# Mirko-Nava/BayesianNeuralNetworks

Measured on AMD Instinct MI355X. Metric: MC-samples/sec (node), 784-1200-1200-10 BayesianLinear MLP, batch 512, higher is better.
Workload: dtype bf16

## Files before the change

### bayesianneuralnetworks_amd/_lib.py

```python
import ctypes
import os

import torch

_HERE = os.path.dirname(os.path.abspath(__file__))
LIB_PATH = os.environ.get("BNN_HIP_LIB") or os.path.join(_HERE, "libbnn_hip.so")

F32, BF16, BF16X3 = 0, 1, 2
DRAW_FLIPOUT = 16
COMPUTE_F32, COMPUTE_BF16 = 0, 1
FLAG_RELU = 1
FLAG_X_BF16 = 2
E_ALIGN, E_UNSUPPORTED, E_DEVICE = -4, -6, -7
FLAG_Y_BF16 = 4
UNC_LOGITS, UNC_PROBS = 0, 1


class BnnHipError(RuntimeError):
    pass


ABI_VERSION = 2


class Rng(ctypes.Structure):
    _fields_ = [("seed", ctypes.c_uint64),
                ("stream", ctypes.c_uint32),
                ("sample0", ctypes.c_uint32),
                ("epoch_host", ctypes.c_uint32),
                ("epoch_dev_delta", ctypes.c_int32),
                ("epoch_dev", ctypes.c_void_p),
                ("generator", ctypes.c_uint32),
                ("reserved", ctypes.c_uint32)]


class KlTensor(ctypes.Structure):
    _fields_ = [("mu", ctypes.c_void_p),
                ("rho", ctypes.c_void_p),
                ("n", ctypes.c_int64),
                ("prior_mu", ctypes.c_float),
                ("prior_sigma", ctypes.c_float)]


class AdamTensor(ctypes.Structure):
    _fields_ = [("p", ctypes.c_void_p), ("g", ctypes.c_void_p), ("m", ctypes.c_void_p), ("v", ctypes.c_void_p),
                ("n", ctypes.c_int64)]


class KlFuse(ctypes.Structure):
    _fields_ = [("upstream", ctypes.c_void_p), ("mu_w", ctypes.c_void_p), ("mu_b", ctypes.c_void_p),
                ("scale_w", ctypes.c_float), ("prior_mu_w", ctypes.c_float), ("prior_sigma_w", ctypes.c_float),
                ("scale_b", ctypes.c_float), ("prior_mu_b", ctypes.c_float), ("prior_sigma_b", ctypes.c_float)]


class DrawTensor(ctypes.Structure):
    _fields_ = [("mu", ctypes.c_void_p), ("rho", ctypes.c_void_p), ("rows", ctypes.c_int64), ("cols", ctypes.c_int64),
                ("out", ctypes.c_void_p), ("ld", ctypes.c_int64), ("out_sample_stride", ctypes.c_int64),
                ("out_dtype", ctypes.c_int), ("kind", ctypes.c_int), ("taps", ctypes.c_int), ("rng", Rng)]


class Conv2dShape(ctypes.Structure):
    _fields_ = [(n, ctypes.c_int32) for n in
                ("B", "C", "H", "W", "O", "KH", "KW", "stride_h", "stride_w", "pad_h", "pad_w",
                 "dil_h", "dil_w", "groups")]


_p = ctypes.c_void_p
_i64 = ctypes.c_int64
_int = ctypes.c_int
_f = ctypes.c_float
_rngp = ctypes.POINTER(Rng)

SIGNATURES = {
    "bnn_abi_version": (_int, []),
    "bnn_arch": (ctypes.c_char_p, []),
    "bnn_last_error": (ctypes.c_char_p, []),
    "bnn_launch_count": (ctypes.c_uint64, []),
    "bnn_set_workspace": (_int, [_int, _p, _i64]),
    "bnn_check_device": (_int, [_int, _p]),
    "bnn_sample_affine_eps": (_int, [_p, _p, _p, _p, _i64, _int, _p]),
    "bnn_sample_affine_philox": (_int, [_p, _p, _p, _i64, _int, _i64, _int, _rngp, _p]),
    "bnn_eps_philox": (_int, [_p, _i64, _int, _i64, _rngp, _p]),
    "bnn_sigma": (_int, [_p, _p, _i64, _p]),
    "bnn_sample_affine_bwd": (_int, [_p, _i64, _p, _p, _i64, _rngp, _i64, _int, _p, _p, _int, _p]),
    "bnn_rng_advance": (_int, [_p, ctypes.c_uint32, _p]),
    "bnn_prune_score": (_int, [_p, _p, _p, _i64, _p]),
    "bnn_kl_workspace_bytes": (_i64, [_int]),
    "bnn_kl_forward": (_int, [ctypes.POINTER(KlTensor), _int, _f, _p, _p, _p]),
    "bnn_kl_forward_partial": (_int, [ctypes.POINTER(KlTensor), _int, _p, _p]),
    "bnn_kl_backward": (_int, [ctypes.POINTER(KlTensor), _int, _f, _p, ctypes.POINTER(_p),
                               ctypes.POINTER(_p), _int, _p]),
    "bnn_linear_forward_sampled": (_int, [_p, _i64, _i64, _p, _p, _p, _p, _p, _i64, _i64, _i64, _i64,
                                          _i64, _int, _rngp, _rngp, _int, _int, _p]),
    "bnn_linear_forward_sampled_kl": (_int, [_p, _i64, _i64, _p, _p, _p, _p, _p, _i64, _i64, _i64, _i64,
                                             _i64, _int, _rngp, _rngp, _int, _int, ctypes.POINTER(KlTensor), _int, _p, _p]),
    "bnn_draw_multi": (_int, [ctypes.POINTER(DrawTensor), _int, _int, ctypes.POINTER(KlTensor), _int, _p, _p]),
    "bnn_dense_forward": (_int, [_p, _i64, _i64, _p, _i64, _i64, _p, _i64, _p, _i64, _i64, _i64, _i64, _i64, _int, _int, _p]),
    "bnn_dense_forward_dropout": (_int, [_p, _i64, _i64, _p, _i64, _i64, _p, _i64, _p, _i64, _i64, _i64, _i64, _i64, _int, _int,
                                         _f, _rngp, _p]),
    "bnn_mc_dropout": (_int, [_p, _i64, _p, _i64, _i64, _i64, _int, _f, _int, _rngp, _p]),
    "bnn_flipout_signs": (_int, [_p, _i64, _i64, _i64, _int, _rngp, _p]),
    "bnn_flipout_weight_backward": (_int, [_p, _i64, _p, _p, _p, _i64, _i64, _int, _rngp, _p]),
    "bnn_mc_dropout_backward": (_int, [_p, _i64, _p, _i64, _i64, _i64, _int, _f, _int, _rngp, _p]),
    "bnn_dense_head_parts": (_int, [_i64, _i64, _int]),
    "bnn_dense_forward_head": (_int, [_p, _i64, _i64, _p, _i64, _i64, _p, _i64, _p, _i64, _i64, _p, _i64, _i64,
                                      _p, _i64, _i64, _i64, _int, _int, _p]),
    "bnn_dense_forward_x3_head": (_int, [_p, _i64, _i64, _i64, _p, _i64, _i64, _i64, _p, _i64, _p, _i64, _i64, _i64,
                                         _p, _i64, _i64, _p, _i64, _i64, _i64, _int, _int, _p]),
    "bnn_dense_forward_x3": (_int, [_p, _i64, _i64, _i64, _p, _i64, _i64, _i64, _p, _i64, _p, _i64, _i64, _i64,
                                    _i64, _i64, _i64, _int, _int, _p]),
    "bnn_split_bf16x3": (_int, [_p, _i64, _i64, _i64, _p, _i64, _i64, _p]),
    "bnn_transpose_bf16": (_int, [_p, _i64, _i64, _p, _i64, _i64, _i64, _i64, _int, _p]),
    "bnn_conv2d_dense_forward_x3": (_int, [_p, _i64, _p, _i64, _i64, _i64, _p, _i64, _p, _i64, ctypes.POINTER(Conv2dShape), _int, _int, _p]),
    "bnn_conv2d_dense_forward": (_int, [_p, _i64, _p, _i64, _i64, _p, _i64, _p, _i64, ctypes.POINTER(Conv2dShape), _int, _int, _p]),
    "bnn_conv2d_flipout_forward": (_int, [_p, _p, _i64, _p, _p, _p, ctypes.POINTER(Conv2dShape), _int, _p]),
    "bnn_conv2d_flipout_forward_mc": (_int, [_p, _i64, _p, _i64, _p, _i64, ctypes.POINTER(Conv2dShape), _int, _rngp, _int, _p]),
    "bnn_conv2d_flipout_forward_x3": (_int, [_p, _p, _i64, _i64, _p, _p, _p, ctypes.POINTER(Conv2dShape), _int, _p]),
    "bnn_linear_forward": (_int, [_p, _i64, _i64, _p, _i64, _p, _i64, _p, _i64, _i64, _i64, _i64, _i64,
                                  _int, _int, _int, _p]),
    "bnn_linear_backward_input_sampled": (_int, [_p, _i64, _i64, _p, _p, _p, _i64, _i64, _i64, _i64, _i64, _int,
                                                 _rngp, _int, _int, _p]),
    "bnn_linear_backward_input": (_int, [_p, _i64, _i64, _p, _i64, _p, _i64, _i64, _i64, _i64, _i64, _int, _int, _p]),
    "bnn_linear_backward_weight_sampled": (_int, [_p, _i64, _i64, _p, _i64, _i64, _p, _p, _p, _p, _p, _p, _i64, _i64,
                                                  _i64, _int, _rngp, _rngp, ctypes.POINTER(KlFuse), _int, _int, _int, _p]),
    "bnn_linear_backward_narrow_sampled": (_int, [_p, _i64, _i64, _p, _i64, _i64, _p, _p, _p, _i64, _i64, _p, _p, _p, _p, _p,
                                                  _i64, _i64, _i64, _int, _rngp, _rngp, ctypes.POINTER(KlFuse), _int, _int, _p]),
    "bnn_linear_backward_weight": (_int, [_p, _i64, _i64, _p, _i64, _i64, _p, _i64, _i64, _i64, _i64, _int, _int,
                                          _int, _int, _p]),
    "bnn_colsum": (_int, [_p, _i64, _i64, _p, _i64, _i64, _int, _int, _p]),
    "bnn_relu_backward": (_int, [_p, _p, _p, _i64, _int, _p]),
    "bnn_adam_step": (_int, [ctypes.POINTER(AdamTensor), _int, _f, _f, _f, _f, _f, _p, _p]),
    "bnn_adam_step_advance": (_int, [ctypes.POINTER(AdamTensor), _int, _f, _f, _f, _f, _f, _p, _p, ctypes.c_uint32, _p]),
    "bnn_xent_workspace_bytes": (_i64, [_i64]),
    "bnn_softmax_xent": (_int, [_p, _p, _i64, _int, _p, _p, _p, _p]),
    "bnn_conv2d_im2col": (_int, [_p, _i64, ctypes.POINTER(Conv2dShape), _int, _p, _int, _p]),
    "bnn_conv2d_col2im": (_int, [_p, ctypes.POINTER(Conv2dShape), _int, _int, _p, _p]),
    "bnn_nchw_to_rows": (_int, [_p, _i64, _int, _int, _p, _int, _p]),
    "bnn_conv2d_workspace_bytes": (_i64, [ctypes.POINTER(Conv2dShape), _int, _int]),
    "bnn_conv2d_forward_sampled": (_int, [_p, _i64, _p, _p, _p, _p, _p, _i64,
                                          ctypes.POINTER(Conv2dShape), _int, _rngp, _rngp, _int, _int, _p, _i64, _p]),
    "bnn_conv2d_forward": (_int, [_p, _i64, _p, _i64, _p, _i64, _p, _i64, ctypes.POINTER(Conv2dShape),
                                  _int, _int, _int, _p, _i64, _p]),
    "bnn_diag_sampler": (_int, [_p, _int, _int, _int, _p]),
    "bnn_diag_astream": (_int, [_p, _int, _int, _int, _int, _int, _int, _int, _p, _p]),
    "bnn_mc_sum": (_int, [_p, _i64, _int, _i64, _f, _p, _int, _p, ctypes.c_uint32, _p]),
    "bnn_mc_sum_kl": (_int, [_p, _i64, _int, _i64, _f, _p, _int, _p, ctypes.c_uint32, ctypes.POINTER(KlTensor), _int, _f,
                             _p, _p, _p]),
    "bnn_mc_uncertainty": (_int, [_p, _i64, _int, _int, _i64, _int, _int, _p, _p, _p, _p, _p, ctypes.c_uint32,
                                  ctypes.POINTER(KlTensor), _int, _f, _p, _p, _p]),
}

_lib = None


def load():
    global _lib
    if _lib is not None:
        return _lib
    if not os.path.exists(LIB_PATH):
        raise BnnHipError(
            "libbnn_hip.so is not built (%s). Run `python -c 'import __graft_entry__ as g; g.build()'` "
            "or `make -C bayesianneuralnetworks_amd/csrc`. There is no fallback path." % LIB_PATH)
    try:
        lib = ctypes.CDLL(LIB_PATH)
    except OSError as e:
        raise BnnHipError("cannot load %s: %s" % (LIB_PATH, e))
    for name, (res, args) in SIGNATURES.items():
        fn = getattr(lib, name)
        fn.restype = res
        fn.argtypes = args
    if lib.bnn_abi_version() != ABI_VERSION:
        raise BnnHipError("libbnn_hip.so has ABI version %d, this package binds version %d (bnn_rng_t carries the generator id "
                          "since version 2): rebuild with `make -C bayesianneuralnetworks_amd/csrc`" % (lib.bnn_abi_version(), ABI_VERSION))
    _lib = _DeviceGuarded(lib)
    return _lib


class _StreamPtr(ctypes.c_void_p):
    device_index = None


class _DeviceGuarded:

    def __init__(self, lib):
        self._lib = lib

    def __getattr__(self, name):
        fn = getattr(self._lib, name)

        def call(*args):
            st = args[-1] if args else None
            if isinstance(st, _StreamPtr) and st.device_index is not None and st.device_index != torch.cuda.current_device():
                with torch.cuda.device(st.device_index):
                    return fn(*args)
            return fn(*args)

        call.__name__ = name
        setattr(self, name, call)
        return call


_workspaces = {}


def ensure_workspace(device):
    idx = device.index if device.index is not None else torch.cuda.current_device()
    if idx not in _workspaces:
        ws = torch.zeros(4 << 20, dtype=torch.uint8, device=torch.device("cuda", idx))
        torch.cuda.synchronize(idx)
        check(load().bnn_set_workspace(idx, ctypes.c_void_p(ws.data_ptr()), ws.numel()), "bnn_set_workspace")
        _workspaces[idx] = ws
    return _workspaces[idx]


def check(rc, what):
    if rc != 0:
        msg = load().bnn_last_error().decode("utf-8", "replace")
        raise BnnHipError("%s failed (code %d): %s" % (what, rc, msg))


def stream_ptr(device=None):
    sp = _StreamPtr(torch.cuda.current_stream(device).cuda_stream)
    if device is not None:
        d = torch.device(device)
        sp.device_index = d.index if d.index is not None else torch.cuda.current_device()
    return sp


def check_device(device=None):
    d = torch.device("cuda", torch.cuda.current_device()) if device is None else torch.device(device)
    idx = d.index if d.index is not None else torch.cuda.current_device()
    check(load().bnn_check_device(idx, stream_ptr(torch.device("cuda", idx))), "bnn_check_device")


def ptr(t):
    if t is None:
        return None
    return ctypes.c_void_p(t.data_ptr())


def require_cuda_act(t, name, contiguous=True):
    if not t.is_cuda:
        raise BnnHipError("%s must be a CUDA/HIP tensor" % name)
    if t.dtype not in (torch.float32, torch.bfloat16):
        raise BnnHipError("%s must be float32 or bfloat16, got %s" % (name, t.dtype))
    if contiguous and not t.is_contiguous():
        raise BnnHipError("%s must be contiguous" % name)


def require_cuda_f32(t, name):
    if not t.is_cuda:
        raise BnnHipError("%s must be a CUDA/HIP tensor" % name)
    if t.dtype != torch.float32:
        raise BnnHipError("%s must be float32, got %s" % (name, t.dtype))
    if not t.is_contiguous():
        raise BnnHipError("%s must be contiguous" % name)
```

### bayesianneuralnetworks_amd/csrc/bnn_dense.hip

```cpp
#include <cstdlib>
#include <type_traits>

#include "bnn_device.hpp"
#include "bnn_dma.hpp"
#include "bnn_kl_body.hpp"

namespace bnn {

typedef float f32x4 __attribute__((ext_vector_type(4)));
typedef __bf16 bf16x8 __attribute__((ext_vector_type(8)));

constexpr int kDrawMaxTensors = 8;
constexpr int kDrawSpreadBelow = 4096;

struct DrawTensorDev {
    const float *mu;
    const float *rho;
    void *out;
    int64_t out_sample_stride;
    int32_t rows, cols, ld;
    int32_t bf16;
    int32_t kind;
    int32_t perm_taps;
    int32_t first_item;
    int32_t spread;
    int32_t flat, pad_first;
    int32_t tapg;
    int32_t kl_on, kl_first;
    float kl_prior_mu, kl_prior_sigma;
    RngDev rng;
};
struct DrawLaunch {
    DrawTensorDev t[kDrawMaxTensors];
    int32_t ntensors;
    int32_t nsamples;
    int32_t total_items;
    int32_t draw_blocks;
    KlPiggy kl;
};

template <int U, bool LEAN>
__device__ __forceinline__ void draw_multi_body(const DrawLaunch &L);

template <int U>
__global__ __launch_bounds__(256) void k_draw_multi(const DrawLaunch L) { draw_multi_body<U, false>(L); }

__global__ __launch_bounds__(256) void k_draw_lean(const DrawLaunch L) { draw_multi_body<1, true>(L); }

template <int U, bool LEAN>
__device__ __forceinline__ void draw_multi_body(const DrawLaunch &L)
{
    if ((int)blockIdx.x < L.kl.nblocks) {
        if (blockIdx.y == 0) kl_piggy_block(L.kl, (int)blockIdx.x);
        return;
    }
    const int item0 = ((int)blockIdx.x - L.kl.nblocks) * 256;
    int ti = 0;
#pragma unroll
    for (int i = 1; i < kDrawMaxTensors; ++i)
        if (i < L.ntensors && item0 >= L.t[i].first_item) ti = i;
    ti = __builtin_amdgcn_readfirstlane(ti);
    const float *const t_mu = L.t[ti].mu;
    const float *const t_rho = L.t[ti].rho;
    char *const t_out = reinterpret_cast<char *>(L.t[ti].out);
    const int64_t t_stride = L.t[ti].out_sample_stride;
    const int t_rows = L.t[ti].rows, t_cols = L.t[ti].cols, t_ld = L.t[ti].ld;
    const bool t_bf16 = L.t[ti].bf16 != 0;
    const bool t_x3 = !LEAN && L.t[ti].bf16 == 2;
    const int t_taps = L.t[ti].perm_taps;
    const int t_kind = L.t[ti].kind;
    const RngDev rng = L.t[ti].rng;
    const int S = L.nsamples;
    int local = item0 + (int)threadIdx.x - L.t[ti].first_item;
    if (L.t[ti].flat) {
        const int esz2 = 2;
        const int64_t sbytes2 = t_stride * esz2, pbytes2 = sbytes2 * S;
        const int padg = (t_ld - t_cols) >> 3;
        if (item0 >= L.t[ti].pad_first) {
            const int pi = item0 + (int)threadIdx.x - L.t[ti].pad_first;
            const int prow = pi / (padg > 0 ? padg : 1);
            if (padg == 0 || prow >= t_rows) return;
            char *d0 = t_out + ((int64_t)prow * t_ld + t_cols + ((pi - prow * padg) << 3)) * esz2;
            for (int s = (int)blockIdx.y; s < S; s += (int)gridDim.y)
                for (int pl = 0; pl < (t_x3 ? 3 : 1); ++pl) *reinterpret_cast<uint4 *>(d0 + s * sbytes2 + pl * pbytes2) = make_uint4(0u, 0u, 0u, 0u);
            return;
        }
        const int64_t e0 = (int64_t)local * 8;
        const bool live = e0 < (int64_t)t_rows * t_cols;
        const uint32_t edev = rng_epoch_dev(rng);
        float4 m0 = make_float4(0.f, 0.f, 0.f, 0.f), m1 = m0, r0 = m0, r1 = m0;
        if (live) {
            m0 = *reinterpret_cast<const float4 *>(t_mu + e0); m1 = *reinterpret_cast<const float4 *>(t_mu + e0 + 4);
            r0 = *reinterpret_cast<const float4 *>(t_rho + e0); r1 = *reinterpret_cast<const float4 *>(t_rho + e0 + 4);
        }
        if (L.t[ti].kl_on && blockIdx.y == 0) {
            const float inv_ps = __uint_as_float(uniform_vgpr(__float_as_uint(1.0f / L.t[ti].kl_prior_sigma)));
            const float pmu = __uint_as_float(uniform_vgpr(__float_as_uint(L.t[ti].kl_prior_mu)));
            float acc = 0.f;
            if (live) {
                acc += kl_elem(m0.x, r0.x, pmu, inv_ps); acc += kl_elem(m0.y, r0.y, pmu, inv_ps);
                acc += kl_elem(m0.z, r0.z, pmu, inv_ps); acc += kl_elem(m0.w, r0.w, pmu, inv_ps);
                acc += kl_elem(m1.x, r1.x, pmu, inv_ps); acc += kl_elem(m1.y, r1.y, pmu, inv_ps);
                acc += kl_elem(m1.z, r1.z, pmu, inv_ps); acc += kl_elem(m1.w, r1.w, pmu, inv_ps);
            }
            kl_block_reduce(acc, L.t[ti].kl_first + ((item0 - L.t[ti].first_item) >> 8), L.kl.partials);
        }
        if (!live) return;
        const int gpc = t_cols >> 3;
        const int row = local / gpc, c0 = (local - row * gpc) << 3;
        const float m[8] = {m0.x, m0.y, m0.z, m0.w, m1.x, m1.y, m1.z, m1.w};
        const float sg[8] = {sigma_draw(r0.x), sigma_draw(r0.y), sigma_draw(r0.z), sigma_draw(r0.w),
                             sigma_draw(r1.x), sigma_draw(r1.y), sigma_draw(r1.z), sigma_draw(r1.w)};
        const PhiloxKeys keys = philox_keys(rng.key0, rng.key1);
        const uint32_t blk = (uint32_t)(e0 >> 2);
        const bool gen16 = LEAN || rng.gen == BNN_GEN_PHILOX7_U16;
        char *dst = t_out + ((int64_t)row * t_ld + c0) * esz2 + (int64_t)blockIdx.y * sbytes2;
        const int64_t step = sbytes2 * (int64_t)gridDim.y;
#pragma unroll U
        for (int s = (int)blockIdx.y; s < S; s += (int)gridDim.y, dst += step) {
            const uint32_t sample = rng.sample0 + (uint32_t)s;
            float4 za, zb;
            if (gen16) {
                eps8_u16(rng, keys, edev, blk >> 1, sample, za, zb);
            } else {
                za = eps4(rng, keys, edev, blk, sample);
                zb = eps4(rng, keys, edev, blk + 1u, sample);
            }
            float w[8];
            w[0] = fmaf(sg[0], za.x, m[0]); w[1] = fmaf(sg[1], za.y, m[1]);
            w[2] = fmaf(sg[2], za.z, m[2]); w[3] = fmaf(sg[3], za.w, m[3]);
            w[4] = fmaf(sg[4], zb.x, m[4]); w[5] = fmaf(sg[5], zb.y, m[5]);
            w[6] = fmaf(sg[6], zb.z, m[6]); w[7] = fmaf(sg[7], zb.w, m[7]);
            if (t_x3) {
                uint4 h, mm, l;
                split_bf16x3(w[0], w[1], h.x, mm.x, l.x); split_bf16x3(w[2], w[3], h.y, mm.y, l.y);
                split_bf16x3(w[4], w[5], h.z, mm.z, l.z); split_bf16x3(w[6], w[7], h.w, mm.w, l.w);
                *reinterpret_cast<uint4 *>(dst) = h;
                *reinterpret_cast<uint4 *>(dst + pbytes2) = mm;
                *reinterpret_cast<uint4 *>(dst + 2 * pbytes2) = l;
            } else {
                uint4 o;
                o.x = pack_bf16x2(w[0], w[1]); o.y = pack_bf16x2(w[2], w[3]);
                o.z = pack_bf16x2(w[4], w[5]); o.w = pack_bf16x2(w[6], w[7]);
                *reinterpret_cast<uint4 *>(dst) = o;
            }
        }
        return;
    }
    if (!LEAN && L.t[ti].tapg) {
        __shared__ __attribute__((aligned(16))) uint16_t timg[3][256 * 8];
        const int taps = t_taps;
        const int ng = 2048 / (8 * taps);
        const int Cn = t_cols / taps, C8 = Cn >> 3;
        const int NG = t_rows * C8;
        const int g0 = ((item0 - L.t[ti].first_item) >> 8) * ng;
        const int i = (int)threadIdx.x;
        const int gl = i / taps, b = i - gl * taps;
// ... 1172 lines not shown
                }
            }
        };
        using I0 = std::integral_constant<int, 0>;
        using I1 = std::integral_constant<int, 1>;
        if (nk_run > 0) {
            __builtin_amdgcn_s_barrier();
            asm volatile("" ::: "memory");
            rd(I0{}, I0{});
            for (int kt = 0; kt + 1 < nk_run; ++kt) {
                rd(I1{}, I1{});
                mm(I0{});
                __builtin_amdgcn_sched_barrier(0);
                asm volatile("s_waitcnt lgkmcnt(0)" ::: "memory");
                __builtin_amdgcn_s_barrier();
                asm volatile("" ::: "memory");
                rd(I0{}, I0{});
                mm(I1{});
                __builtin_amdgcn_sched_barrier(0);
            }
            rd(I1{}, I1{});
            mm(I0{});
            mm(I1{});
        }
    }

    __syncthreads();
    float *T = reinterpret_cast<float *>(lds);
    if constexpr (KEYED) {
        const float *rs = reinterpret_cast<const float *>(lds + LDSB) - NSX * p.IMG * p.O;
#pragma unroll
        for (int n = 0; n < NSX; ++n) {
            if (n >= nvalid) break;
            if (n > 0) __syncthreads();
            if (wave < NWV) {
#pragma unroll
                for (int b = 0; b < TO; ++b) {
                    const int o = b * 16 + fi;
#pragma unroll
                    for (int a = 0; a < TM; ++a) {
                        const int row0 = wave * WM + a * 16 + fq * 4;
                        int il = row0 / P, pix = row0 - il * P;
#pragma unroll
                        for (int r = 0; r < 4; ++r) {
                            if (row0 + r < imgs * P && o < p.O)
                                T[(il * p.O + o) * P + pix] = fmaf(rs[(n * p.IMG + il) * p.O + o], acc[a][TO + n * TO + b][r], acc[a][b][r]);
                            if (++pix == P) { pix = 0; ++il; }
                        }
                    }
                }
            }
            __syncthreads();
            float *Yt = p.Y + (int64_t)(s + n) * p.y_sample_stride + (int64_t)b0 * p.O * P;
            const int nn = (p.flags & 4) ? 0 : imgs * p.O * P;
            if ((nn & 3) == 0 && (reinterpret_cast<uintptr_t>(Yt) & 15u) == 0) {
                for (int i = tid; i < (nn >> 2); i += 512) reinterpret_cast<uint4 *>(Yt)[i] = reinterpret_cast<const uint4 *>(T)[i];
            } else {
                for (int i = tid; i < nn; i += 512) Yt[i] = T[i];
            }
        }
        return;
    }
    if (wave < NWV) {
        const float *bias = p.bias ? p.bias + (int64_t)s * p.bias_sample_stride : nullptr;
#pragma unroll
        for (int b = 0; b < NOUT / 16; ++b) {
            const int o = b * 16 + fi;
            const float bv = (bias && o < p.O) ? bias[o] : 0.f;
#pragma unroll
            for (int a = 0; a < TM; ++a) {
                const int row0 = wave * WM + a * 16 + fq * 4;
                int il = row0 / P, pix = row0 - il * P;
#pragma unroll
                for (int r = 0; r < 4; ++r) {
                    if (row0 + r < imgs * P && o < p.O) {
                        float v = acc[a][b][r] + bv;
                        if constexpr (FLIP) v = fmaf(p.sgn_out[(int64_t)(b0 + il) * p.O + o], acc[a][b + TN / 2][r], v);
                        T[(il * p.O + o) * P + pix] = v;
                    }
                    if (++pix == P) { pix = 0; ++il; }
                }
            }
        }
    }
    __syncthreads();
    {
        float *Yt = p.Y + (int64_t)s * p.y_sample_stride + (int64_t)b0 * p.O * P;
        const int n = (p.flags & 4) ? 0 : imgs * p.O * P;
        if ((n & 3) == 0 && (reinterpret_cast<uintptr_t>(Yt) & 15u) == 0) {
            for (int i = tid; i < (n >> 2); i += 512) reinterpret_cast<uint4 *>(Yt)[i] = reinterpret_cast<const uint4 *>(T)[i];
        } else {
            for (int i = tid; i < n; i += 512) Yt[i] = T[i];
        }
    }
}

static inline bool al16(const void *q) { return (reinterpret_cast<uintptr_t>(q) & 15u) == 0; }

}

using namespace bnn;

namespace bnn {
__global__ __launch_bounds__(256) void k_split_bf16x3(const float *__restrict__ x, int gpr, int64_t ldx, uint16_t *__restrict__ out,
                                                     int64_t ld_out, int64_t plane_stride, int items)
{
    const int i = (int)(blockIdx.x * 256 + threadIdx.x);
    if (i >= items) return;
    const int row = i / gpr, c0 = (i - row * gpr) * 8;
    const float4 a = *reinterpret_cast<const float4 *>(x + (int64_t)row * ldx + c0);
    const float4 b = *reinterpret_cast<const float4 *>(x + (int64_t)row * ldx + c0 + 4);
    uint4 h, m, l;
    split_bf16x3(a.x, a.y, h.x, m.x, l.x);
    split_bf16x3(a.z, a.w, h.y, m.y, l.y);
    split_bf16x3(b.x, b.y, h.z, m.z, l.z);
    split_bf16x3(b.z, b.w, h.w, m.w, l.w);
    uint16_t *o = out + (int64_t)row * ld_out + c0;
    *reinterpret_cast<uint4 *>(o) = h;
    *reinterpret_cast<uint4 *>(o + plane_stride) = m;
    *reinterpret_cast<uint4 *>(o + 2 * plane_stride) = l;
}

__global__ __launch_bounds__(256) void k_transpose_bf16(const uint16_t *__restrict__ in, int64_t in_batch_stride, int64_t ld_in,
                                                       uint16_t *__restrict__ out, int64_t out_batch_stride, int64_t ld_out,
                                                       int rows, int cols)
{
    constexpr int PITCH = 72;
    __shared__ __attribute__((aligned(16))) uint16_t T[64 * PITCH];
    const int r0 = (int)blockIdx.x * 64, c0 = (int)blockIdx.y * 64;
    const uint16_t *src = in + (int64_t)blockIdx.z * in_batch_stride;
    uint16_t *dst = out + (int64_t)blockIdx.z * out_batch_stride;
#pragma unroll
    for (int j = 0; j < 2; ++j) {
        const int q = (int)threadIdx.x + 256 * j;
        const int r = q >> 3, cc = (q & 7) * 8;
        uint4 v = make_uint4(0u, 0u, 0u, 0u);
        if (r0 + r < rows && c0 + cc < cols) v = *reinterpret_cast<const uint4 *>(src + (int64_t)(r0 + r) * ld_in + c0 + cc);
        const uint32_t e[4] = {v.x, v.y, v.z, v.w};
#pragma unroll
        for (int i = 0; i < 4; ++i) {
            T[(cc + 2 * i) * PITCH + r] = (uint16_t)(e[i] & 0xFFFFu);
            T[(cc + 2 * i + 1) * PITCH + r] = (uint16_t)(e[i] >> 16);
        }
    }
    __syncthreads();
#pragma unroll
    for (int j = 0; j < 2; ++j) {
        const int q = (int)threadIdx.x + 256 * j;
        const int c = q >> 3, rc = (q & 7) * 8;
        if (c0 + c < cols && r0 + rc < ld_out)
            *reinterpret_cast<uint4 *>(dst + (int64_t)(c0 + c) * ld_out + r0 + rc) = *reinterpret_cast<const uint4 *>(&T[c * PITCH + rc]);
    }
}
}

struct HeadArgs {
    const void *wh;
    int64_t wh_plane_stride;
    int64_t wh_sample_stride, ldwh;
    const float *bh;
    int64_t bh_sample_stride;
    float *partials;
    int64_t nh;
};

struct DropArgs {
    float p;
    const bnn_rng_t *rng;
    bool fan;
};

static int dense_pick_tile(int64_t M, int64_t N, int nsamples)
{
    static const int force_tile = [] { const char *e = getenv("BNN_DENSE_TILE"); return e ? atoi(e) : -1; }();
    int tile = (N % 80 == 0 || N < 128) ? 1 : 2;
    if (N <= 80) tile = 0;
    if (force_tile >= 0 && force_tile <= 4) tile = force_tile;
    if (tile == 1 && force_tile < 0) {
        const int64_t cols = (N + 159) / 160;
        if (((M + 127) / 128) * cols * nsamples < 128 && M > 64) tile = 3;
        if (tile == 3 && ((M + 63) / 64) * cols * nsamples < 128 && M > 32) tile = 4;
    }
    return tile;
}

static int dense_launch(const char *who, const void *x, int64_t x_plane_stride, int64_t x_sample_stride, int64_t ldx,
                        const void *w, int64_t w_plane_stride, int64_t w_sample_stride, int64_t ldw,
                        const float *b, int64_t b_sample_stride,
                        void *y, int64_t y_plane_stride, int64_t y_sample_stride, int64_t ldy,
                        int64_t M, int64_t N, int64_t K, int nsamples, int flags, bool x3, void *stream, const HeadArgs *head = nullptr,
                        const DropArgs *drop = nullptr)
{
    if (M == 0 && N >= 1 && K >= 1 && nsamples >= 1) return BNN_OK;
    if (head) { y = head->partials; ldy = N; }
    if (!x || !w || !y) { set_error("%s: NULL pointer", who); return BNN_E_NULL; }
    if (M < 0 || N < 1 || K < 1 || nsamples < 1 || ldx < K || ldy < N) { set_error("%s: bad extent", who); return BNN_E_SHAPE; }
    if (M > 0x7FFFFFFF || N > 0x7FFFFFFF || K > 0x7FFFFFFF) { set_error("%s: extent too large", who); return BNN_E_RANGE; }
    if (flags & ~(BNN_FLAG_RELU | BNN_FLAG_Y_BF16)) { set_error("%s: unknown flags", who); return BNN_E_UNSUPPORTED; }
    const int64_t kp = (K + 63) / 64 * 64;
    if (K % 8 != 0 || ldx % 8 != 0 || x_sample_stride % 8 != 0 || ldw % 8 != 0 || w_sample_stride % 8 != 0 || ldw < kp || !al16(x) || !al16(w)) {
        set_error("%s: needs K %% 8 == 0, 16-B aligned bf16 rows, and weight rows zero-padded to ldw >= roundup(K, 64)", who);
        return BNN_E_UNSUPPORTED;
    }
    if (M * ldx * 2 >= ((int64_t)1 << 32) || N * ldw * 2 >= ((int64_t)1 << 32)) { set_error("%s: one sample's operand exceeds 4 GiB", who); return BNN_E_RANGE; }
    const bool ybf = (flags & BNN_FLAG_Y_BF16) != 0;
    if (reinterpret_cast<uintptr_t>(y) & (ybf ? 1u : 3u)) { set_error("%s: misaligned output", who); return BNN_E_ALIGN; }
    DenseParams p{};
    p.A = reinterpret_cast<const uint16_t *>(x); p.a_sample_stride = x_sample_stride; p.lda = ldx;
    p.W = reinterpret_cast<const uint16_t *>(w); p.w_sample_stride = w_sample_stride; p.ldw = ldw;
    p.bias = b; p.bias_sample_stride = b_sample_stride;
    p.Y = y; p.y_sample_stride = y_sample_stride; p.ldy = ldy;
    p.M = (int32_t)M; p.N = (int32_t)N; p.K = (int32_t)K; p.S = nsamples; p.flags = flags;
    if (x3) {
        if (x_plane_stride % 8 != 0 || w_plane_stride % 8 != 0 || (ybf && y_plane_stride % 8 != 0) || x_plane_stride < M * ldx || w_plane_stride < N * ldw) {
            set_error("%s: bad plane stride", who);
            return BNN_E_SHAPE;
        }
        if (N <= 16 && (K > 4 * kHeadMaxSteps * 32 || ybf)) { set_error("%s: a narrow layer (N <= 16) on three-plane operands needs K <= %d and fp32 outputs", who, 4 * kHeadMaxSteps * 32); return BNN_E_UNSUPPORTED; }
        p.x3 = 1;
        p.a_plane_stride = x_plane_stride; p.w_plane_stride = w_plane_stride; p.y_plane_stride = y_plane_stride;
    }
    if (head) {
        if (N <= 16 || (flags & BNN_FLAG_Y_BF16) == 0) { set_error("%s: the fused head follows a hidden layer wider than 16", who); return BNN_E_UNSUPPORTED; }
        if (x3 && (head->wh_plane_stride % 8 != 0 || head->wh_plane_stride < head->nh * head->ldwh)) { set_error("%s: bad plane stride of the head's weights", who); return BNN_E_SHAPE; }
        if (x3) {
            const int t_ = dense_pick_tile(M, N, nsamples);
            if (t_ == 0 || t_ == 2) { set_error("%s: the three-plane fused head runs on the 160-column tiles (N %% 80 == 0 or N < 128, N > 80)", who); return BNN_E_UNSUPPORTED; }
        }
        if (!head->wh || head->nh < 1 || head->nh > 16) { set_error("%s: head of 1 .. 16 outputs", who); return BNN_E_SHAPE; }
        if (N % 8 != 0 || head->ldwh % 8 != 0 || head->ldwh < N || head->wh_sample_stride % 8 != 0 || !al16(head->wh) ||
            (reinterpret_cast<uintptr_t>(head->partials) & 3u)) {
            set_error("%s: the head's weights need N %% 8 == 0 and 16-B aligned rows zero-padded to ldwh >= N", who);
            return BNN_E_UNSUPPORTED;
        }
        p.Wh = reinterpret_cast<const uint16_t *>(head->wh); p.wh_sample_stride = head->wh_sample_stride; p.ldwh = head->ldwh;
        p.bias_h = head->bh; p.bias_h_sample_stride = head->bh_sample_stride;
        p.P = head->partials; p.Nh = (int32_t)head->nh;
        p.wh_plane_stride = head->wh_plane_stride;
    }
    hipStream_t st = (hipStream_t)stream;
    const int full_samples = nsamples;
    if (drop) {
        if (x3 || head) { set_error("%s: the dropout epilogue takes plain bf16 operands", who); return BNN_E_UNSUPPORTED; }
        p.drop_rng = make_rng(drop->rng);
        p.drop_p = drop->p;
        p.drop_scale = drop->p < 1.f ? 1.f / (1.f - drop->p) : 0.f;
        p.drop_fan = drop->fan ? nsamples : 1;
        if (drop->fan) nsamples = p.S = 1;
    }
    if (N <= 16 && K <= 4 * kHeadMaxSteps * 32) {
        p.ntm = (int32_t)((M + 15) / 16);
        p.ntn = 1;
        hipLaunchKernelGGL(k_head_bf16, dim3((unsigned)((int64_t)p.ntm * nsamples)), dim3(256), 0, st, p);
        int rc = check_launch(who);
        if (rc == BNN_OK && drop)
            rc = mc_dropout_launch(who, y, drop->fan ? 0 : y_sample_stride, ldy, y, y_sample_stride, ldy, M, N, full_samples, drop->fan,
                                   drop->p, ybf ? BNN_BF16 : BNN_F32, drop->rng, st);
        return rc;
    }
    const bool fused_drop = drop && N % 4 == 0;
    static const bool no_xcd = [] { const char *e = getenv("BNN_DENSE_XCD"); return e && e[0] == '0'; }();
    if (no_xcd) p.flags |= kDenseNoXcdMap;
    static const bool lprio = [] { const char *e = getenv("BNN_DENSE_LOADER_PRIO"); return e && e[0] == '1'; }();
    if (lprio) p.flags |= kDenseLoaderPrio;
    int tile = dense_pick_tile(M, N, nsamples);
    if (fused_drop && tile == 2) tile = 1;
    const int bm = tile == 1 ? 128 : tile == 3 ? 64 : tile == 4 ? 32 : 256;
    const int bn = tile == 0 ? 80 : tile == 2 ? 128 : 160;
    p.ntm = (int32_t)((M + bm - 1) / bm);
    p.ntn = (int32_t)((N + bn - 1) / bn);
    const int64_t grid = (int64_t)p.ntm * p.ntn * nsamples;
    if (grid > 0x7FFFFFFF) { set_error("%s: grid too large", who); return BNN_E_RANGE; }
    static const int diag = [] { const char *e = getenv("BNN_DENSE_DIAG"); return e ? atoi(e) : 0; }();
    if (diag >= 6 && diag <= 9 && !head && !drop) {
        static const uint64_t stamps = [] { const char *e = getenv("BNN_DENSE_STAMPS"); return e ? strtoull(e, nullptr, 0) : 0ull; }();
        p.P = reinterpret_cast<float *>(stamps);
    }
    const bool relu = (flags & BNN_FLAG_RELU) != 0;
    const dim3 g((unsigned)grid), blk(512);
#define BNN_DENSE_LAUNCH(TM_, TN_, NWM_, NWN_, ST_, RELU_, DROP_) \
    do { \
        if (fused_drop && ybf) hipLaunchKernelGGL((k_dense_bf16<TM_, TN_, NWM_, NWN_, ST_, 1, RELU_, 0, DROP_>), g, blk, 0, st, p); \
        else if (fused_drop) hipLaunchKernelGGL((k_dense_bf16<TM_, TN_, NWM_, NWN_, ST_, 0, RELU_, 0, DROP_>), g, blk, 0, st, p); \
        else if (head) hipLaunchKernelGGL((k_dense_bf16<TM_, TN_, NWM_, NWN_, ST_, 3, RELU_>), g, blk, 0, st, p); \
        else if (x3 && ybf) hipLaunchKernelGGL((k_dense_bf16<TM_, TN_, NWM_, NWN_, ST_, 2, RELU_>), g, blk, 0, st, p); \
        else if (!ybf) hipLaunchKernelGGL((k_dense_bf16<TM_, TN_, NWM_, NWN_, ST_, 0, RELU_>), g, blk, 0, st, p); \
        else if (diag == 1) hipLaunchKernelGGL((k_dense_bf16<TM_, TN_, NWM_, NWN_, ST_, 1, RELU_, 1>), g, blk, 0, st, p); \
        else if (diag == 2) hipLaunchKernelGGL((k_dense_bf16<TM_, TN_, NWM_, NWN_, ST_, 1, RELU_, 2>), g, blk, 0, st, p); \
        else if (diag == 3) hipLaunchKernelGGL((k_dense_bf16<TM_, TN_, NWM_, NWN_, ST_, 1, RELU_, 3>), g, blk, 0, st, p); \
        else if (diag == 4) hipLaunchKernelGGL((k_dense_bf16<TM_, TN_, NWM_, NWN_, ST_, 1, RELU_, 4>), g, blk, 0, st, p); \
        else if (diag == 5) hipLaunchKernelGGL((k_dense_bf16<TM_, TN_, NWM_, NWN_, ST_, 1, RELU_, 5>), g, blk, 0, st, p); \
        else if (diag == 6) hipLaunchKernelGGL((k_dense_bf16<TM_, TN_, NWM_, NWN_, ST_, 1, RELU_, 6>), g, blk, 0, st, p); \
        else if (diag == 7) hipLaunchKernelGGL((k_dense_bf16<TM_, TN_, NWM_, NWN_, ST_, 1, RELU_, 7>), g, blk, 0, st, p); \
        else if (diag == 8) hipLaunchKernelGGL((k_dense_bf16<TM_, TN_, NWM_, NWN_, ST_, 1, RELU_, 8>), g, blk, 0, st, p); \
        else if (diag == 9) hipLaunchKernelGGL((k_dense_bf16<TM_, TN_, NWM_, NWN_, ST_, 1, RELU_, 9>), g, blk, 0, st, p); \
        else hipLaunchKernelGGL((k_dense_bf16<TM_, TN_, NWM_, NWN_, ST_, 1, RELU_>), g, blk, 0, st, p); \
    } while (0)
#define BNN_DENSE_PICK(TM_, TN_, NWM_, NWN_, ST_, DROP_) \
    do { \
        if (relu) BNN_DENSE_LAUNCH(TM_, TN_, NWM_, NWN_, ST_, true, DROP_); else BNN_DENSE_LAUNCH(TM_, TN_, NWM_, NWN_, ST_, false, DROP_); \
    } while (0)
    if (tile == 0) BNN_DENSE_PICK(4, 5, 4, 1, 3, true);
    else if (tile == 1) BNN_DENSE_PICK(4, 5, 2, 2, 4, true);
    else if (tile == 3) BNN_DENSE_PICK(2, 5, 2, 2, 4, true);
    else if (tile == 4) BNN_DENSE_PICK(1, 5, 2, 2, 4, true);
    else BNN_DENSE_PICK(4, 8, 4, 1, 3, false);
#undef BNN_DENSE_PICK
#undef BNN_DENSE_LAUNCH
    int rc = check_launch(who);
    if (rc == BNN_OK && drop && !fused_drop)
        rc = mc_dropout_launch(who, y, drop->fan ? 0 : y_sample_stride, ldy, y, y_sample_stride, ldy, M, N, full_samples, drop->fan,
                               drop->p, ybf ? BNN_BF16 : BNN_F32, drop->rng, st);
    return rc;
}


extern "C" {

int bnn_draw_multi(const bnn_draw_tensor_t *tensors, int ntensors, int nsamples,
                   const bnn_kl_tensor_t *kl_tensors, int kl_ntensors, void *kl_workspace, void *stream)
{
    const char *who = "bnn_draw_multi";
    if (!tensors) { set_error("%s: NULL tensors", who); return BNN_E_NULL; }
    if (ntensors < 1 || ntensors > kDrawMaxTensors) { set_error("%s: 1 .. %d tensors per call", who, kDrawMaxTensors); return BNN_E_RANGE; }
    if (nsamples < 1) { set_error("%s: nsamples < 1", who); return BNN_E_SHAPE; }
    DrawLaunch L{};
    L.ntensors = ntensors;
    L.nsamples = nsamples;
    int64_t items = 0;
    for (int i = 0; i < ntensors; ++i) {
        const bnn_draw_tensor_t &t = tensors[i];
        if (!t.mu || !t.rho || !t.out) { set_error("%s: tensor %d: NULL pointer", who, i); return BNN_E_NULL; }
        if (t.rows < 1 || t.cols < 1 || t.ld < t.cols || t.rows > 0x7FFFFFFF || t.ld > 0x7FFFFFFF) { set_error("%s: tensor %d: bad extent", who, i); return BNN_E_SHAPE; }
        if (t.out_dtype != BNN_F32 && t.out_dtype != BNN_BF16 && t.out_dtype != BNN_BF16X3) { set_error("%s: tensor %d: unknown dtype", who, i); return BNN_E_DTYPE; }
        if (t.rows > 1 && t.cols % 4 != 0) { set_error("%s: tensor %d: cols %% 4 != 0 (use bnn_sample_affine_philox)", who, i); return BNN_E_UNSUPPORTED; }
        if (t.ld % 8 != 0 && t.rows > 1) { set_error("%s: tensor %d: ld %% 8 != 0", who, i); return BNN_E_UNSUPPORTED; }
        if (t.out_dtype != BNN_F32 && (!al16(t.out) || t.out_sample_stride % 8 != 0 || t.ld % 8 != 0)) { set_error("%s: tensor %d: bf16 output needs 16-B aligned rows", who, i); return BNN_E_ALIGN; }
        if ((reinterpret_cast<uintptr_t>(t.mu) | reinterpret_cast<uintptr_t>(t.rho) | reinterpret_cast<uintptr_t>(t.out)) & 3u) { set_error("%s: tensor %d: misaligned pointer", who, i); return BNN_E_ALIGN; }
        const int rc = (t.kind == 0 || t.kind == BNN_DRAW_FLIPOUT) ? check_rng(&t.rng, nsamples) : BNN_OK;
        if (rc) { set_error("%s: tensor %d: bad rng", who, i); return rc; }
        DrawTensorDev &d = L.t[i];
        d.mu = t.mu; d.rho = t.rho; d.out = t.out; d.out_sample_stride = t.out_sample_stride;
        d.rows = (int32_t)t.rows; d.cols = (int32_t)t.cols; d.ld = (int32_t)t.ld; d.bf16 = t.out_dtype == BNN_BF16 ? 1 : t.out_dtype == BNN_BF16X3 ? 2 : 0;
        d.perm_taps = t.taps > 1 ? t.taps : 1;
        d.kind = t.kind;
        if ((t.kind < 0 || t.kind > 3) && t.kind != BNN_DRAW_FLIPOUT) { set_error("%s: tensor %d: kind must be 0 (draw), 1 (mean), 2 (stddev), 3 (as it is, once) or BNN_DRAW_FLIPOUT", who, i); return BNN_E_RANGE; }
        if (t.kind == BNN_DRAW_FLIPOUT && (t.taps > 1 || t.out_dtype == BNN_BF16X3 || t.rows + t.cols > 0xFFFFFFFFll)) { set_error("%s: tensor %d: a Flipout draw is a linear weight (no taps, fp32 or bf16 output, rows + cols < 2^32)", who, i); return BNN_E_SHAPE; }
        if (t.taps > 1 && (t.cols % t.taps != 0 || t.out_dtype == BNN_F32)) { set_error("%s: tensor %d: taps must divide cols (bf16 or three-plane output)", who, i); return BNN_E_SHAPE; }
        d.first_item = (int32_t)items;
        d.rng = make_rng(&t.rng);
        const int64_t nit = t.rows * ((t.ld + 7) / 8);
        d.spread = (nit < kDrawSpreadBelow && nsamples > 1 && nit * nsamples <= 0x7FFFFFFF) ? 1 : 0;
        d.flat = (!d.spread && t.out_dtype != BNN_F32 && t.kind == 0 && t.taps <= 1 && t.cols % 8 == 0 && t.ld % 8 == 0 && al16(t.mu) && al16(t.rho)) ? 1 : 0;
        d.tapg = (t.taps > 1 && t.taps <= 256 && t.out_dtype != BNN_F32 && t.rows >= 1 && (t.cols / t.taps) % 8 == 0 && t.ld % 8 == 0 &&
                  al16(t.mu) && (t.kind == 1 || t.kind == 3 || al16(t.rho))) ? 1 : 0;
        static const bool no_tapg = [] { const char *e = getenv("BNN_DRAW_TAPG"); return e && e[0] == '0'; }();
        if (no_tapg) d.tapg = 0;
        if (d.tapg) {
            d.spread = 0;
            const int64_t ng = 2048 / (8 * t.taps), NG = t.rows * (t.cols / t.taps / 8);
            items += (NG + ng - 1) / ng * 256;
        } else if (d.flat) {
            items += (t.rows * (t.cols / 8) + 255) / 256 * 256;
            d.pad_first = (int32_t)items;
            items += (t.rows * ((t.ld - t.cols) / 8) + 255) / 256 * 256;
        } else
        items += ((d.spread ? nit * nsamples : nit) + 255) / 256 * 256;
        if (items > 0x7FFFFF00) { set_error("%s: too many elements for one call", who); return BNN_E_RANGE; }
    }
    L.total_items = (int32_t)items;
    L.draw_blocks = (int32_t)((items + 255) / 256);
    int64_t grid = L.draw_blocks;
    if (kl_tensors && kl_ntensors > 0) {
        if (!kl_plan_piggy(kl_tensors, kl_ntensors, kl_workspace, L.kl)) {
            set_error("%s: the KL first pass cannot ride along (more than %d tensors, bad prior or no workspace): launch bnn_kl_forward_partial", who, kKlPiggyMax);
            return BNN_E_UNSUPPORTED;
        }
        static const bool kl_items = [] { const char *e = getenv("BNN_DRAW_KL_ITEMS"); return !(e && e[0] == '0'); }();
        int32_t launched = 0;
        for (int j = 0; j < kl_ntensors; ++j) {
            const int32_t nb = L.kl.pg_first[j + 1] - L.kl.pg_first[j];
            bool in_items = false;
            for (int i = 0; i < ntensors && kl_items && !in_items; ++i) {
                DrawTensorDev &d = L.t[i];
                if (d.flat && !d.kl_on && d.mu == kl_tensors[j].mu && d.rho == kl_tensors[j].rho &&
                    kl_tensors[j].n == (int64_t)d.rows * d.cols) {
                    d.kl_on = 1; d.kl_first = L.kl.t[j].first_block;
                    d.kl_prior_mu = kl_tensors[j].prior_mu; d.kl_prior_sigma = kl_tensors[j].prior_sigma;
                    in_items = true;
                }
            }
            L.kl.pg_first[j] = launched;
            if (!in_items) launched += nb;
        }
        L.kl.pg_first[kl_ntensors] = launched;
        L.kl.nblocks = launched;
        grid += L.kl.nblocks;
    }
    int split = 1;
    while (split < nsamples && (int64_t)L.draw_blocks * split < 1024) split *= 2;
    if (split > nsamples) split = nsamples;
    static const int force_split = [] { const char *e = getenv("BNN_DRAW_SPLIT"); return e ? atoi(e) : 0; }();
    if (force_split >= 1 && force_split <= nsamples) split = force_split;
    static const int unroll = [] { const char *e = getenv("BNN_DRAW_UNROLL"); return e ? atoi(e) : 1; }();
    bool lean = true;
    for (int i = 0; i < ntensors; ++i) {
        const DrawTensorDev &d = L.t[i];
        if (d.tapg || d.perm_taps > 1 || d.bf16 == 2 || d.kind == BNN_DRAW_FLIPOUT || (d.kind == 0 && d.rng.gen != BNN_GEN_PHILOX7_U16)) lean = false;
    }
    static const bool no_lean = [] { const char *e = getenv("BNN_DRAW_LEAN"); return e && e[0] == '0'; }();
    if (lean && !no_lean && unroll <= 1) hipLaunchKernelGGL(k_draw_lean, dim3((unsigned)grid, (unsigned)split), dim3(256), 0, (hipStream_t)stream, L);
    else if (unroll == 2) hipLaunchKernelGGL(k_draw_multi<2>, dim3((unsigned)grid, (unsigned)split), dim3(256), 0, (hipStream_t)stream, L);
    else if (unroll == 4) hipLaunchKernelGGL(k_draw_multi<4>, dim3((unsigned)grid, (unsigned)split), dim3(256), 0, (hipStream_t)stream, L);
    else if (unroll == 8) hipLaunchKernelGGL(k_draw_multi<8>, dim3((unsigned)grid, (unsigned)split), dim3(256), 0, (hipStream_t)stream, L);
    else
    hipLaunchKernelGGL(k_draw_multi<1>, dim3((unsigned)grid, (unsigned)split), dim3(256), 0, (hipStream_t)stream, L);
    return check_launch(who);
}

int bnn_dense_forward(const void *x, int64_t x_sample_stride, int64_t ldx,
                      const void *w, int64_t w_sample_stride, int64_t ldw,
                      const float *b, int64_t b_sample_stride,
                      void *y, int64_t y_sample_stride, int64_t ldy,
                      int64_t M, int64_t N, int64_t K, int nsamples, int flags, void *stream)
{
    return dense_launch("bnn_dense_forward", x, 0, x_sample_stride, ldx, w, 0, w_sample_stride, ldw, b, b_sample_stride,
                        y, 0, y_sample_stride, ldy, M, N, K, nsamples, flags, false, stream);
}

int bnn_dense_forward_dropout(const void *x, int64_t x_sample_stride, int64_t ldx,
                              const void *w, int64_t w_sample_stride, int64_t ldw,
                              const float *b, int64_t b_sample_stride,
                              void *y, int64_t y_sample_stride, int64_t ldy,
                              int64_t M, int64_t N, int64_t K, int nsamples, int flags, float p, const bnn_rng_t *rng, void *stream)
{
    const char *who = "bnn_dense_forward_dropout";
    if (!x || !w || !y) { set_error("%s: NULL pointer", who); return BNN_E_NULL; }
    int rc = check_dropout_args(who, M, N, nsamples, p, rng);
    if (rc) return rc;
    if (x_sample_stride < 0 || w_sample_stride < 0 || b_sample_stride < 0 || y_sample_stride < 0 ||
        (nsamples > 1 && y_sample_stride < (M - 1) * ldy + N)) { set_error("%s: bad sample stride", who); return BNN_E_SHAPE; }
    const DropArgs d{p, rng, x_sample_stride == 0 && w_sample_stride == 0 && (b == nullptr || b_sample_stride == 0)};
    return dense_launch(who, x, 0, x_sample_stride, ldx, w, 0, w_sample_stride, ldw, b, b_sample_stride,
                        y, 0, y_sample_stride, ldy, M, N, K, nsamples, flags, false, stream, nullptr, &d);
}

int bnn_dense_head_parts(int64_t M, int64_t N, int nsamples)
{
    if (M < 1 || N < 17 || nsamples < 1) return 0;
    const int tile = dense_pick_tile(M, N, nsamples);
    const int bn = tile == 0 ? 80 : tile == 2 ? 128 : 160;
    const int nwn = (tile == 0 || tile == 2) ? 1 : 2;
    return (int)((N + bn - 1) / bn) * nwn;
}

int bnn_dense_forward_head(const void *x, int64_t x_sample_stride, int64_t ldx,
                           const void *w, int64_t w_sample_stride, int64_t ldw,
                           const float *b, int64_t b_sample_stride,
                           const void *w_head, int64_t wh_sample_stride, int64_t ldwh,
                           const float *b_head, int64_t bh_sample_stride, int64_t n_head,
                           float *partials, int64_t M, int64_t N, int64_t K, int nsamples, int flags, void *stream)
{
    HeadArgs h{w_head, 0, wh_sample_stride, ldwh, b_head, bh_sample_stride, partials, n_head};
    return dense_launch("bnn_dense_forward_head", x, 0, x_sample_stride, ldx, w, 0, w_sample_stride, ldw, b, b_sample_stride,
                        nullptr, 0, 0, N, M, N, K, nsamples, flags | BNN_FLAG_Y_BF16, false, stream, &h);
}

int bnn_dense_forward_x3_head(const void *x, int64_t x_plane_stride, int64_t x_sample_stride, int64_t ldx,
                              const void *w, int64_t w_plane_stride, int64_t w_sample_stride, int64_t ldw,
                              const float *b, int64_t b_sample_stride,
                              const void *w_head, int64_t wh_plane_stride, int64_t wh_sample_stride, int64_t ldwh,
                              const float *b_head, int64_t bh_sample_stride, int64_t n_head,
                              float *partials, int64_t M, int64_t N, int64_t K, int nsamples, int flags, void *stream)
{
    if (wh_plane_stride <= 0) { set_error("bnn_dense_forward_x3_head: plane stride of the head's weights"); return BNN_E_SHAPE; }
    HeadArgs h{w_head, wh_plane_stride, wh_sample_stride, ldwh, b_head, bh_sample_stride, partials, n_head};
    return dense_launch("bnn_dense_forward_x3_head", x, x_plane_stride, x_sample_stride, ldx, w, w_plane_stride, w_sample_stride, ldw,
                        b, b_sample_stride, nullptr, 0, 0, N, M, N, K, nsamples, flags | BNN_FLAG_Y_BF16, true, stream, &h);
}

int bnn_dense_forward_x3(const void *x, int64_t x_plane_stride, int64_t x_sample_stride, int64_t ldx,
                         const void *w, int64_t w_plane_stride, int64_t w_sample_stride, int64_t ldw,
                         const float *b, int64_t b_sample_stride,
                         void *y, int64_t y_plane_stride, int64_t y_sample_stride, int64_t ldy,
                         int64_t M, int64_t N, int64_t K, int nsamples, int flags, void *stream)
{
    return dense_launch("bnn_dense_forward_x3", x, x_plane_stride, x_sample_stride, ldx, w, w_plane_stride, w_sample_stride, ldw,
                        b, b_sample_stride, y, y_plane_stride, y_sample_stride, ldy, M, N, K, nsamples, flags, true, stream);
}

int bnn_split_bf16x3(const float *x, int64_t rows, int64_t cols, int64_t ldx, void *out, int64_t ld_out, int64_t plane_stride, void *stream)
{
    const char *who = "bnn_split_bf16x3";
    if (rows == 0 && cols >= 1) return BNN_OK;
    if (!x || !out) { set_error("%s: NULL pointer", who); return BNN_E_NULL; }
    if (rows < 0 || cols < 1 || ldx < cols || ld_out < cols) { set_error("%s: bad extent", who); return BNN_E_SHAPE; }
    if (cols % 8 != 0 || ldx % 4 != 0 || ld_out % 8 != 0 || plane_stride % 8 != 0 || !al16(x) || !al16(out)) {
        set_error("%s: needs cols %% 8 == 0 and 16-B aligned rows on both sides", who);
        return BNN_E_UNSUPPORTED;
    }
    const int64_t items = rows * (cols / 8);
    if (items > 0x7FFFFFFF) { set_error("%s: too many elements", who); return BNN_E_RANGE; }
    hipLaunchKernelGGL(k_split_bf16x3, dim3((unsigned)((items + 255) / 256)), dim3(256), 0, (hipStream_t)stream,
                       x, (int)(cols / 8), ldx, reinterpret_cast<uint16_t *>(out), ld_out, plane_stride, (int)items);
    return check_launch(who);
}

int bnn_transpose_bf16(const void *in, int64_t in_batch_stride, int64_t ld_in, void *out, int64_t out_batch_stride, int64_t ld_out,
                       int64_t rows, int64_t cols, int batch, void *stream)
{
    const char *who = "bnn_transpose_bf16";
    if ((rows == 0 || batch == 0) && cols >= 1) return BNN_OK;
    if (!in || !out) { set_error("%s: NULL pointer", who); return BNN_E_NULL; }
    if (rows < 0 || cols < 1 || batch < 0 || ld_in < cols || ld_out < rows) { set_error("%s: bad extent", who); return BNN_E_SHAPE; }
    if (cols % 8 != 0 || ld_in % 8 != 0 || ld_out % 8 != 0 || in_batch_stride % 8 != 0 || out_batch_stride % 8 != 0 || !al16(in) || !al16(out)) {
        set_error("%s: needs cols %% 8 == 0 and 16-B aligned rows on both sides", who);
        return BNN_E_UNSUPPORTED;
    }
    if (rows > 0x7FFFFFFF || cols > 0x7FFFFFFF || (cols + 63) / 64 > 65535 || batch > 65535) { set_error("%s: extent too large", who); return BNN_E_RANGE; }
    hipLaunchKernelGGL(k_transpose_bf16, dim3((unsigned)((ld_out + 63) / 64), (unsigned)((cols + 63) / 64), (unsigned)batch), dim3(256), 0,
                       (hipStream_t)stream, reinterpret_cast<const uint16_t *>(in), in_batch_stride, ld_in,
                       reinterpret_cast<uint16_t *>(out), out_batch_stride, ld_out, (int)rows, (int)cols);
    return check_launch(who);
}


}

static int conv_dense_launch(const float *x, int64_t x_sample_stride, const void *w, int64_t w_sample_stride, int64_t ldw,
                             const float *b, int64_t b_sample_stride, const float *sgn_in, const float *sgn_out,
                             float *y, int64_t y_sample_stride, const bnn_conv2d_shape_t *sh, int nsamples, int flags,
                             void *stream, const char *who, int64_t w_plane_stride = 0, const bnn_rng_t *rng = nullptr)
{
    const bool keyed = rng != nullptr;
    const bool flip = sgn_in != nullptr || keyed;
    const bool x3 = w_plane_stride != 0;
    if (!x || !w || !y || !sh || (flip && !keyed && !sgn_out)) { set_error("%s: NULL pointer", who); return BNN_E_NULL; }
    if (sh->B < 1 || sh->C < 1 || sh->H < 1 || sh->W < 1 || sh->O < 1 || sh->KH < 1 || sh->KW < 1 || sh->stride_h < 1 ||
        sh->stride_w < 1 || sh->pad_h < 0 || sh->pad_w < 0 || sh->dil_h < 1 || sh->dil_w < 1 || nsamples < 1) { set_error("%s: bad shape", who); return BNN_E_SHAPE; }
    if (flags != 0) { set_error("%s: unknown flags", who); return BNN_E_UNSUPPORTED; }
    const int OH = (sh->H + 2 * sh->pad_h - sh->dil_h * (sh->KH - 1) - 1) / sh->stride_h + 1;
    const int OW = (sh->W + 2 * sh->pad_w - sh->dil_w * (sh->KW - 1) - 1) / sh->stride_w + 1;
    if (OH < 1 || OW < 1) { set_error("%s: kernel larger than the padded input", who); return BNN_E_SHAPE; }
    const int K = sh->C * sh->KH * sh->KW;
    const int bn = flip ? 2 * sh->O : sh->O;
    const bool ok = sh->groups == 1 && (sh->C == 64 || sh->C % 128 == 0) && (bn == 64 || bn == 128) &&
                    ldw >= K && ldw % 8 == 0 && w_sample_stride % 8 == 0 && al16(w) &&
                    (reinterpret_cast<uintptr_t>(x) & 3u) == 0 && (reinterpret_cast<uintptr_t>(y) & 3u) == 0;
    if (!ok) { set_error("%s: needs groups = 1, C = 64 or a multiple of 128, O = 64 or 128 (Flipout: 32 or 64), tap-major bf16 weights with 16-B aligned rows", who); return BNN_E_UNSUPPORTED; }
    const int ns = !keyed ? 0 : (x_sample_stride != 0 || nsamples == 1) ? 1 : (nsamples == 2 || bn == 128) ? 2 : 4;
    if (keyed) {
        const int rc = check_flip_args(who, sh->B, (int64_t)sh->O + sh->C, nsamples, rng);
        if (rc) return rc;
    }
    ConvParams p{};
    const int64_t img_bytes = (int64_t)sh->H * sh->W * sh->C * 2 + (flip ? (sh->C / 8) * 16 * (keyed ? ns : 1) : 0);
    const int64_t rsign = keyed ? (int64_t)ns * sh->O * 4 : 0;
    const int P = OH * OW;
    if (x3 && (w_plane_stride % 8 != 0 || w_plane_stride < (int64_t)bn * ldw)) { set_error("%s: bad plane stride", who); return BNN_E_SHAPE; }
    const int st = bn == 64 ? 4 : (x3 ? 3 : flip ? 4 : 6);
    const int64_t lds_block = (bn == 64 && !x3 && !keyed) ? kConvLds : kConvLdsBig;
    const int64_t ring = (int64_t)st * bn * 128;
    int img = 128 / P;
    while (img > 0 && (img * (img_bytes * (x3 ? 3 : 1) + rsign) + ring > lds_block || (int64_t)img * (sh->O * P * 4 + rsign) > lds_block)) --img;
    if (img > sh->B) img = sh->B;
    if (img < 1 || (int64_t)bn * ldw * 2 >= ((int64_t)1 << 32)) { set_error("%s: one image (%lld B bf16) + the weight ring do not fit the LDS block, or more than 128 output pixels per image", who, (long long)img_bytes); return BNN_E_UNSUPPORTED; }
    p.X = x; p.x_sample_stride = x_sample_stride;
    p.W = reinterpret_cast<const uint16_t *>(w); p.w_sample_stride = w_sample_stride; p.ldw = ldw;
    p.bias = b; p.bias_sample_stride = b_sample_stride;
    p.Y = y; p.y_sample_stride = y_sample_stride;
    p.sgn_in = sgn_in; p.sgn_out = sgn_out;
    p.w_plane_stride = w_plane_stride;
    p.B = sh->B; p.C = sh->C; p.H = sh->H; p.Wd = sh->W; p.O = sh->O; p.KH = sh->KH; p.KW = sh->KW;
    p.sh = sh->stride_h; p.sw = sh->stride_w; p.ph = sh->pad_h; p.pw = sh->pad_w; p.dh = sh->dil_h; p.dw = sh->dil_w;
    static const int cdiag = [] { const char *e = getenv("BNN_CONV_DIAG"); return e ? atoi(e) : 0; }();
    p.flags = cdiag;
    p.OH = OH; p.OW = OW; p.S = nsamples; p.IMG = img; p.ntiles = (sh->B + img - 1) / img;
    p.img_bytes = (int32_t)((int64_t)sh->H * sh->W * sh->C * 2);
    if (keyed) p.rng = make_rng(rng);
    const int64_t grid = (int64_t)p.ntiles * (keyed ? (nsamples + ns - 1) / ns : nsamples);
    if (grid > 0x7FFFFFFF) { set_error("%s: grid too large", who); return BNN_E_RANGE; }
    const dim3 g((unsigned)grid), blk(512);
    hipStream_t stq = (hipStream_t)stream;
    if (keyed) {
        if (bn == 64) {
            if (ns == 1) hipLaunchKernelGGL((k_conv_bf16<4, 4, kConvLdsBig, true, false, 1>), g, blk, 0, stq, p);
            else if (ns == 2) hipLaunchKernelGGL((k_conv_bf16<4, 4, kConvLdsBig, true, false, 2>), g, blk, 0, stq, p);
            else hipLaunchKernelGGL((k_conv_bf16<4, 4, kConvLdsBig, true, false, 4>), g, blk, 0, stq, p);
        } else {
            if (ns == 1) hipLaunchKernelGGL((k_conv_bf16<8, 4, kConvLdsBig, true, false, 1>), g, blk, 0, stq, p);
            else hipLaunchKernelGGL((k_conv_bf16<8, 4, kConvLdsBig, true, false, 2>), g, blk, 0, stq, p);
        }
    } else if (x3 && flip) {
        if (bn == 64) hipLaunchKernelGGL((k_conv_bf16<4, 4, kConvLdsBig, true, true>), g, blk, 0, stq, p);
        else hipLaunchKernelGGL((k_conv_bf16<8, 3, kConvLdsBig, true, true>), g, blk, 0, stq, p);
    } else if (x3) {
        if (bn == 64) hipLaunchKernelGGL((k_conv_bf16<4, 4, kConvLdsBig, false, true>), g, blk, 0, stq, p);
        else hipLaunchKernelGGL((k_conv_bf16<8, 3, kConvLdsBig, false, true>), g, blk, 0, stq, p);
    } else if (flip) {
        if (bn == 64) hipLaunchKernelGGL((k_conv_bf16<4, 4, kConvLds, true>), g, blk, 0, stq, p);
        else hipLaunchKernelGGL((k_conv_bf16<8, 4, kConvLdsBig, true>), g, blk, 0, stq, p);
    } else {
        if (bn == 64) hipLaunchKernelGGL((k_conv_bf16<4, 4, kConvLds>), g, blk, 0, stq, p);
        else hipLaunchKernelGGL((k_conv_bf16<8, 6, kConvLdsBig>), g, blk, 0, stq, p);
    }
    return check_launch(who);
}

extern "C" {

int bnn_conv2d_dense_forward(const float *x, int64_t x_sample_stride,
                             const void *w, int64_t w_sample_stride, int64_t ldw,
                             const float *b, int64_t b_sample_stride,
                             float *y, int64_t y_sample_stride,
                             const bnn_conv2d_shape_t *sh, int nsamples, int flags, void *stream)
{
    return conv_dense_launch(x, x_sample_stride, w, w_sample_stride, ldw, b, b_sample_stride, nullptr, nullptr, y, y_sample_stride,
                             sh, nsamples, flags, stream, "bnn_conv2d_dense_forward");
}

int bnn_conv2d_dense_forward_x3(const float *x, int64_t x_sample_stride,
                                const void *w, int64_t w_plane_stride, int64_t w_sample_stride, int64_t ldw,
                                const float *b, int64_t b_sample_stride,
                                float *y, int64_t y_sample_stride,
                                const bnn_conv2d_shape_t *sh, int nsamples, int flags, void *stream)
{
    if (w_plane_stride <= 0) { set_error("bnn_conv2d_dense_forward_x3: plane stride"); return BNN_E_SHAPE; }
    return conv_dense_launch(x, x_sample_stride, w, w_sample_stride, ldw, b, b_sample_stride, nullptr, nullptr, y, y_sample_stride,
                             sh, nsamples, flags, stream, "bnn_conv2d_dense_forward_x3", w_plane_stride);
}

int bnn_conv2d_flipout_forward(const float *x, const void *w, int64_t ldw, const float *sign_in, const float *sign_out,
                               float *y, const bnn_conv2d_shape_t *sh, int flags, void *stream)
{
    if (!sign_in || !sign_out) { set_error("bnn_conv2d_flipout_forward: NULL sign tensor"); return BNN_E_NULL; }
    return conv_dense_launch(x, 0, w, 0, ldw, nullptr, 0, sign_in, sign_out, y, 0, sh, 1, flags, stream, "bnn_conv2d_flipout_forward");
}

int bnn_conv2d_flipout_forward_mc(const float *x, int64_t x_sample_stride, const void *w, int64_t ldw, float *y,
                                  int64_t y_sample_stride, const bnn_conv2d_shape_t *sh, int nsamples, const bnn_rng_t *rng,
                                  int flags, void *stream)
{
    const char *who = "bnn_conv2d_flipout_forward_mc";
// ... 22 lines not shown
```

### bayesianneuralnetworks_amd/csrc/bnn_gemm.hip

```cpp
#include <cstdlib>

#include "bnn_device.hpp"
#include "bnn_gemm_params.hpp"

namespace bnn {

typedef float f32x4 __attribute__((ext_vector_type(4)));
typedef __bf16 bf16x8 __attribute__((ext_vector_type(8)));

__device__ __forceinline__ int swz(int row, int chunk)
{
    return chunk ^ ((0x78 >> (((row >> 2) & 3) * 2)) & 3);
}

template <int BM, int BN, int WM, int WN, int A_MODE, int B_MODE, int COMPUTE>
__global__ __launch_bounds__(WM * WN * 64) void k_gemm_nt(const GemmParams p)
{
    constexpr int NT = WM * WN * 64;
    constexpr int KPC = (COMPUTE == BNN_COMPUTE_F32) ? 4 : 8;
    constexpr int BK = 4 * KPC;
    constexpr int WTM = BM / WM, WTN = BN / WN;
    constexpr int TM = WTM / 16, TN = WTN / 16;
    static_assert(WTM % 16 == 0 && WTN % 16 == 0, "wave tile must be a multiple of 16x16");
    constexpr int A_CHUNKS = BM * 4, B_CHUNKS = BN * 4;
// ... 177 lines not shown
                Bs[row * 4 + swz(row, c)] = pack(bm[i]);
            }
        }
    };

    f32x4 acc[TM][TN];
#pragma unroll
    for (int a = 0; a < TM; ++a)
#pragma unroll
        for (int b = 0; b < TN; ++b) acc[a][b] = f32x4{0.f, 0.f, 0.f, 0.f};

    const int nk = (p.K + BK - 1) / BK;
    const int fi = lane & 15, fq = lane >> 4;

    load_A(0);
    load_B(0);
    sample_B(0);
    store_tiles(0);
    __syncthreads();

    for (int kt = 0; kt < nk; ++kt) {
        const int buf = kt & 1;
        const bool more = kt + 1 < nk;
        if (more) {
            load_A((kt + 1) * BK);
            load_B((kt + 1) * BK);
        }
        const uint4 *As = As0 + buf * A_CHUNKS, *Bs = Bs0 + buf * B_CHUNKS;
        uint4 af[TM], bf[TN];
#pragma unroll
        for (int a = 0; a < TM; ++a) {
            const int row = wm * WTM + a * 16 + fi;
            af[a] = As[row * 4 + swz(row, fq)];
        }
#pragma unroll
        for (int b = 0; b < TN; ++b) {
            const int row = wn * WTN + b * 16 + fi;
            bf[b] = Bs[row * 4 + swz(row, fq)];
        }
        if constexpr (COMPUTE == BNN_COMPUTE_F32) {
#pragma unroll
            for (int j = 0; j < 4; ++j)
#pragma unroll
                for (int a = 0; a < TM; ++a)
#pragma unroll
                    for (int b = 0; b < TN; ++b) {
                        const uint32_t ua = j == 0 ? af[a].x : j == 1 ? af[a].y : j == 2 ? af[a].z : af[a].w;
                        const uint32_t ub = j == 0 ? bf[b].x : j == 1 ? bf[b].y : j == 2 ? bf[b].z : bf[b].w;
                        acc[a][b] = __builtin_amdgcn_mfma_f32_16x16x4f32(__uint_as_float(ua), __uint_as_float(ub),
                                                                         acc[a][b], 0, 0, 0);
                    }
        } else {
#pragma unroll
            for (int a = 0; a < TM; ++a)
#pragma unroll
                for (int b = 0; b < TN; ++b)
                    acc[a][b] = __builtin_amdgcn_mfma_f32_16x16x32_bf16(__builtin_bit_cast(bf16x8, af[a]),
                                                                        __builtin_bit_cast(bf16x8, bf[b]),
                                                                        acc[a][b], 0, 0, 0);
        }
        if (more) {
            sample_B((kt + 1) * BK);
            store_tiles(buf ^ 1);
        }
        __syncthreads();
    }

    uint32_t edev_b = 0;
    const bool sampled_bias = (p.mu_b != nullptr);
    if (sampled_bias) edev_b = rng_epoch_dev(p.rng_b);
#pragma unroll
    for (int b = 0; b < TN; ++b) {
        const int n = n0 + wn * WTN + b * 16 + fi;
        if (n >= p.N) continue;
        const int64_t ng = nrow0 + n;
        float bias = 0.f;
        if (sampled_bias)
            bias = fmaf(sigma_draw(p.rho_b[ng]), eps1(p.rng_b, edev_b, (uint64_t)ng, p.rng_b.sample0 + (uint32_t)s), p.mu_b[ng]);
        else if (p.bias)
            bias = p.bias[(int64_t)s * p.bias_sample_stride + ng];
#pragma unroll
        for (int a = 0; a < TM; ++a) {
#pragma unroll
            for (int r = 0; r < 4; ++r) {
                const int m = m0 + wm * WTM + a * 16 + fq * 4 + r;
                if (m >= p.M) continue;
                float v = acc[a][b][r] + bias;
                if (p.flags & BNN_FLAG_RELU) v = fmaxf(v, 0.f);
                float *Yb = p.Y + (int64_t)s * p.y_sample_stride;
                if constexpr (A_MODE == A_DENSE) {
                    Yb[(int64_t)m * p.ldy + ng] = v;
                } else {
                    const int hw = p.OH * p.OW;
                    const int bimg = m / hw, pix = m % hw;
                    Yb[((int64_t)bimg * p.O + ng) * hw + pix] = v;
                }
            }
        }
    }
}

struct TileCfg { int bm, bn; };

template <int BM, int BN, int WM, int WN, int AM, int BMODE, int CP>
static void launch_cfg(GemmParams &p, hipStream_t st)
{
    p.ntm = (p.M + BM - 1) / BM;
    p.ntn = (p.N + BN - 1) / BN;
    const int panels = p.ntn * p.G;
    const int64_t grid = (int64_t)8 * ((panels + 7) / 8) * p.ntm * p.S;
    hipLaunchKernelGGL((k_gemm_nt<BM, BN, WM, WN, AM, BMODE, CP>), dim3((unsigned)grid), dim3(WM * WN * 64), 0, st, p);
}

template <int AM, int BMODE, int CP>
static void launch_select(GemmParams &p, hipStream_t st)
{
    const int64_t tiles_big = (int64_t)((p.M + 255) / 256) * ((p.N + 79) / 80) * p.S * p.G;
    if (p.N <= 16) {
        launch_cfg<64, 16, 4, 1, AM, BMODE, CP>(p, st);
    } else if (p.M >= 256 && p.N >= 80 && tiles_big >= 128) {
        launch_cfg<256, 80, 8, 1, AM, BMODE, CP>(p, st);
    } else {
        launch_cfg<64, 64, 2, 2, AM, BMODE, CP>(p, st);
    }
}

template <int AM>
static int dispatch(GemmParams &p, bool sampled, int compute, hipStream_t st, const char *who)
{
    if (compute == BNN_COMPUTE_F32) {
        if (sampled) launch_select<AM, B_SAMPLED, BNN_COMPUTE_F32>(p, st);
        else launch_select<AM, B_PLAIN, BNN_COMPUTE_F32>(p, st);
    } else if (compute == BNN_COMPUTE_BF16) {
        if (sampled) launch_select<AM, B_SAMPLED, BNN_COMPUTE_BF16>(p, st);
        else launch_select<AM, B_PLAIN, BNN_COMPUTE_BF16>(p, st);
    } else {
        set_error("%s: unknown compute mode %d", who, compute);
        return BNN_E_DTYPE;
    }
    return check_launch(who);
}

static void *g_ws[64];
static int64_t g_ws_bytes[64];
constexpr int64_t kTicketBytes = 64 * 1024;

void fill_workspace(GemmParams &p)
{
    int dev = 0;
    if (hipGetDevice(&dev) != hipSuccess || dev < 0 || dev >= 64 || !g_ws[dev] || g_ws_bytes[dev] <= kTicketBytes) return;
    p.dev_err = reinterpret_cast<unsigned *>(g_ws[dev]);
    p.ws_slabs = reinterpret_cast<float *>(reinterpret_cast<char *>(g_ws[dev]) + kTicketBytes);
    p.ws_slab_bytes = g_ws_bytes[dev] - kTicketBytes;
}

static inline bool al16(const void *q) { return (reinterpret_cast<uintptr_t>(q) & 15u) == 0; }
static inline bool al4(const void *q) { return (reinterpret_cast<uintptr_t>(q) & 3u) == 0; }

static int linear_common(const float *x, int64_t x_sample_stride, int64_t ldx,
                         const float *w, int64_t w_sample_stride, const float *b, int64_t b_sample_stride,
                         const float *mu_w, const float *rho_w, const float *mu_b, const float *rho_b,
                         float *y, int64_t y_sample_stride, int64_t ldy, int64_t M, int64_t N, int64_t K,
                         int nsamples, const bnn_rng_t *rng_w, const bnn_rng_t *rng_b, bool sampled,
                         int compute, int flags, void *stream, const char *who, KlPiggy *kl = nullptr)
{
    if (M == 0 && N >= 1 && K >= 1 && nsamples >= 1) return BNN_OK;
    if (!x || !y || (sampled ? (!mu_w || !rho_w) : !w)) { set_error("%s: NULL pointer", who); return BNN_E_NULL; }
    if (sampled && ((mu_b == nullptr) != (rho_b == nullptr))) { set_error("%s: mu_b / rho_b must both be given or both NULL", who); return BNN_E_NULL; }
    if (M < 0 || N < 1 || K < 1 || nsamples < 1 || ldx < K || ldy < N) { set_error("%s: bad extent (M=%lld N=%lld K=%lld S=%d ldx=%lld ldy=%lld)", who, (long long)M, (long long)N, (long long)K, nsamples, (long long)ldx, (long long)ldy); return BNN_E_SHAPE; }
    if (M > 0x7FFFFFFF || N > 0x7FFFFFFF || K > 0x7FFFFFFF || N * K > ((int64_t)1 << 34)) { set_error("%s: extent too large", who); return BNN_E_RANGE; }
    const bool xh = (flags & BNN_FLAG_X_BF16) != 0, yh = (flags & BNN_FLAG_Y_BF16) != 0;
    if (!(xh ? (reinterpret_cast<uintptr_t>(x) & 1u) == 0 : al4(x)) || !(yh ? (reinterpret_cast<uintptr_t>(y) & 1u) == 0 : al4(y))) { set_error("%s: misaligned pointer", who); return BNN_E_ALIGN; }
    if (xh || yh) {
        const bool ok = compute == BNN_COMPUTE_BF16 && (K % 4 == 0) &&
                        (!xh || (al16(x) && K % 8 == 0 && ldx % 8 == 0 && x_sample_stride % 8 == 0)) &&
                        (xh || (al16(x) && ldx % 4 == 0 && x_sample_stride % 4 == 0)) &&
                        (sampled ? (al16(mu_w) && al16(rho_w)) : (al16(w) && w_sample_stride % 4 == 0));
        if (!ok) { set_error("%s: BNN_FLAG_X_BF16 / Y_BF16 need bf16 compute, 16-B aligned operands, K %% 8 == 0", who); return BNN_E_UNSUPPORTED; }
    }
    if (sampled) {
        int rc = check_rng(rng_w, nsamples);
        if (rc) { set_error("%s: bad rng_w", who); return rc; }
        if (mu_b) { rc = check_rng(rng_b, nsamples); if (rc) { set_error("%s: bad rng_b", who); return rc; } }
    }
    if (M == 0) return BNN_OK;
    GemmParams p{};
    p.A = x; p.a_sample_stride = x_sample_stride; p.lda = ldx;
    p.Bw = w; p.b_sample_stride = w_sample_stride; p.mu = mu_w; p.rho = rho_w;
    p.bias = sampled ? nullptr : b; p.bias_sample_stride = b_sample_stride;
    p.mu_b = sampled ? mu_b : nullptr; p.rho_b = sampled ? rho_b : nullptr;
    p.Y = y; p.y_sample_stride = y_sample_stride; p.ldy = ldy; p.O = (int32_t)N;
    p.M = (int32_t)M; p.N = (int32_t)N; p.K = (int32_t)K; p.S = nsamples; p.G = 1; p.flags = flags;
    p.vecA = xh ? 1 : (al16(x) && (ldx % 4 == 0) && (x_sample_stride % 4 == 0));
    p.vecB = (K % 4 == 0) && (sampled ? (al16(mu_w) && al16(rho_w)) : (al16(w) && w_sample_stride % 4 == 0));
    if (sampled) { p.rng_w = make_rng(rng_w); p.rng_b = make_rng(mu_b ? rng_b : nullptr); }
    static const bool force_v1 = [] { const char *e = getenv("BNN_LINEAR_KERNEL"); return e && e[0] == 'v' && e[1] == '1'; }();
    if (p.vecA && p.vecB && !force_v1) {
        fill_workspace(p);
        if (kl) p.kl = *kl;
        const int rc = dispatch_linear_v2(p, sampled, compute, (hipStream_t)stream, who);
        if (kl) kl->taken = p.kl.taken;
        return rc;
    }
    return dispatch<A_DENSE>(p, sampled, compute, (hipStream_t)stream, who);
}

template <bool BF>
__global__ __launch_bounds__(256) void k_im2col(const float *__restrict__ x, int64_t x_sample_stride, void *__restrict__ out,
                                                int B, int C, int H, int W, int OH, int OW, int KH, int KW,
                                                int sh_, int sw_, int ph, int pw, int dh, int dw, int K, int64_t groups8)
{
    const int KQ = K / 8, P = OH * OW, KHW = KH * KW;
    for (int64_t id = (int64_t)blockIdx.x * 256 + threadIdx.x; id < groups8; id += (int64_t)gridDim.x * 256) {
        const int kg = (int)(id % KQ);
        const int64_t mrow = id / KQ;
        const int s = (int)(mrow / ((int64_t)B * P));
        const int ml = (int)(mrow % ((int64_t)B * P));
        const int b = ml / P, pix = ml % P;
        const int oh = pix / OW, ow = pix % OW;
        int k = kg * 8;
        int c = k / KHW, rem = k % KHW;
        int kh = rem / KW, kw = rem % KW;
        const float *xb = x + (int64_t)s * x_sample_stride + (int64_t)b * C * H * W;
        float v[8];
#pragma unroll
        for (int j = 0; j < 8; ++j) {
            const int ih = oh * sh_ - ph + kh * dh, iw = ow * sw_ - pw + kw * dw;
            v[j] = (ih >= 0 && ih < H && iw >= 0 && iw < W) ? xb[((int64_t)c * H + ih) * W + iw] : 0.f;
            if (++kw == KW) { kw = 0; if (++kh == KH) { kh = 0; ++c; } }
        }
        if constexpr (BF) {
            uint4 o;
            o.x = pack_bf16x2(v[0], v[1]); o.y = pack_bf16x2(v[2], v[3]);
            o.z = pack_bf16x2(v[4], v[5]); o.w = pack_bf16x2(v[6], v[7]);
            *reinterpret_cast<uint4 *>(reinterpret_cast<uint16_t *>(out) + mrow * K + k) = o;
        } else {
            float *q = reinterpret_cast<float *>(out) + mrow * K + k;
            *reinterpret_cast<float4 *>(q) = make_float4(v[0], v[1], v[2], v[3]);
            *reinterpret_cast<float4 *>(q + 4) = make_float4(v[4], v[5], v[6], v[7]);
        }
    }
}

__device__ __forceinline__ void fdivmod(int n, int d, float inv_d, int &q, int &r)
{
    q = (int)((float)n * inv_d);
    r = n - q * d;
    if (r < 0) { r += d; --q; }
    if (r >= d) { r -= d; ++q; }
}

template <bool BF>
__global__ __launch_bounds__(256) void k_im2col_img(const float *__restrict__ x, int64_t x_sample_stride, void *__restrict__ out,
                                                    int B, int C, int H, int W, int OH, int OW, int KH, int KW,
                                                    int sh_, int sw_, int ph, int pw, int dh, int dw, int K,
                                                    float inv_KQ, float inv_OW, float inv_KHW, float inv_KW)
{
    extern __shared__ float img[];
    const int chw = C * H * W, P = OH * OW, KQ = K / 8, KHW = KH * KW;
    const int s = blockIdx.x / B, b = blockIdx.x % B;
    const float *xb = x + (int64_t)s * x_sample_stride + (int64_t)b * chw;
    if ((chw & 3) == 0 && (reinterpret_cast<uintptr_t>(xb) & 15u) == 0) {
        for (int i = threadIdx.x; i < chw / 4; i += 256) reinterpret_cast<float4 *>(img)[i] = reinterpret_cast<const float4 *>(xb)[i];
    } else {
        for (int i = threadIdx.x; i < chw; i += 256) img[i] = xb[i];
    }
    __syncthreads();
    const int64_t row0 = (int64_t)blockIdx.x * P;
    for (int oct = threadIdx.x; oct < P * KQ; oct += 256) {
        int pix, kg, oh, ow, c, rem, kh, kw;
        fdivmod(oct, KQ, inv_KQ, pix, kg);
        fdivmod(pix, OW, inv_OW, oh, ow);
        const int k = kg * 8;
        fdivmod(k, KHW, inv_KHW, c, rem);
        fdivmod(rem, KW, inv_KW, kh, kw);
        float v[8];
#pragma unroll
        for (int j = 0; j < 8; ++j) {
            const int ih = oh * sh_ - ph + kh * dh, iw = ow * sw_ - pw + kw * dw;
            v[j] = (ih >= 0 && ih < H && iw >= 0 && iw < W) ? img[(c * H + ih) * W + iw] : 0.f;
            if (++kw == KW) { kw = 0; if (++kh == KH) { kh = 0; ++c; } }
        }
        const int64_t o = (row0 + pix) * K + k;
        if constexpr (BF) {
            uint4 q;
            q.x = pack_bf16x2(v[0], v[1]); q.y = pack_bf16x2(v[2], v[3]);
            q.z = pack_bf16x2(v[4], v[5]); q.w = pack_bf16x2(v[6], v[7]);
            *reinterpret_cast<uint4 *>(reinterpret_cast<uint16_t *>(out) + o) = q;
        } else {
            float *q = reinterpret_cast<float *>(out) + o;
            *reinterpret_cast<float4 *>(q) = make_float4(v[0], v[1], v[2], v[3]);
            *reinterpret_cast<float4 *>(q + 4) = make_float4(v[4], v[5], v[6], v[7]);
        }
    }
}

static void launch_im2col(const float *x, int64_t x_sample_stride, void *panel, const bnn_conv2d_shape_t *sh, int64_t OH, int64_t OW,
                          int64_t K, int nsx, int64_t M, bool bf, hipStream_t st)
{
    const int64_t rows = (int64_t)nsx * M;
    {
        const int64_t chw = (int64_t)sh->C * sh->H * sh->W, P = OH * OW, images = (int64_t)nsx * sh->B;
        if (chw * 4 <= 64 * 1024 && P * (K / 8) < (1 << 22) && K < (1 << 22) && images <= 0x7FFFFFFF) {
            const unsigned lds = (unsigned)(chw * 4);
            const float iKQ = 1.0f / (float)(K / 8), iOW = 1.0f / (float)OW, iKHW = 1.0f / (float)(sh->KH * sh->KW), iKW = 1.0f / (float)sh->KW;
            if (bf) hipLaunchKernelGGL((k_im2col_img<true>), dim3((unsigned)images), dim3(256), lds, st, x, x_sample_stride, panel, sh->B, sh->C, sh->H, sh->W, (int)OH, (int)OW, sh->KH, sh->KW, sh->stride_h, sh->stride_w, sh->pad_h, sh->pad_w, sh->dil_h, sh->dil_w, (int)K, iKQ, iOW, iKHW, iKW);
// ... 325 lines not shown
```

### bayesianneuralnetworks_amd/csrc/bnn_gemm_params.hpp

```cpp
#pragma once
#include "bnn_device.hpp"
#include "bnn_kl_body.hpp"

namespace bnn {

enum { A_DENSE = 0, A_IM2COL = 1 };
enum { B_PLAIN = 0, B_SAMPLED = 1, B_SAMPLED_T = 2 };

constexpr int kFlagStoreNCHW = 1 << 16;
constexpr unsigned kDevErrHandoffTimeout = 1u;
constexpr int kComputeBf16x3 = 2;

struct GemmParams {
    const float *A;
    int64_t a_sample_stride;
    int64_t lda;
    int32_t C, H, W, OH, OW, KH, KW, sh, sw, ph, pw, dh, dw, Cg;
    const float *Bw;
    int64_t b_sample_stride;
    const float *mu;
    const float *rho;
    const float *bias;
    int64_t bias_sample_stride;
    const float *mu_b;
    const float *rho_b;
    float *Y;
    int64_t y_sample_stride;
    int64_t ldy;
    int32_t O;
    int32_t M, N, K;
    int32_t S, G;
    int32_t ntn, ntm;
    int32_t xcd_a;
    int32_t flags;
    int32_t vecA, vecB;
    RngDev rng_w, rng_b;
    unsigned *dev_err;
    float *ws_slabs;
    int64_t ws_slab_bytes;
    KlPiggy kl;
    int32_t gemm_grid;
    unsigned long long *dbg;
    int32_t dbg_block;
};

int dispatch_linear_v2(GemmParams &p, bool sampled, int compute, hipStream_t st, const char *who);
int dispatch_linear_dgrad(GemmParams &p, int compute, hipStream_t st, const char *who);
void fill_workspace(GemmParams &p);

}
```

### bayesianneuralnetworks_amd/nn/_settings.py

```python
_default = "f32"


def set_compute(mode):
    global _default
    if mode not in ("f32", "bf16"):
        raise ValueError("compute mode must be 'f32' or 'bf16'")
    _default = mode


def get_compute():
    return _default


def fuse_kl_gradient(enable=True):
    from .. import ops
    ops.FUSE_KL_GRADIENT = bool(enable)


def fuse_activations(module, bf16_activations=False, fuse_head=False):
    import torch
    from .dense import NormalLinear
    fused = 0
    for m in module.modules():
        if isinstance(m, torch.nn.Sequential):
            names = list(m._modules.keys())
            for a, b in zip(names[:-1], names[1:]):
                la, lb = m._modules[a], m._modules[b]
                if type(la) is NormalLinear and type(lb) is torch.nn.ReLU and la.activation is None:
                    la.activation = 'relu'
                    m._modules[b] = torch.nn.Identity()
                    fused += 1
            if bf16_activations:
                mods = [m._modules[n] for n in names]
                for i, la in enumerate(mods):
                    if type(la) is NormalLinear and la.activation == 'relu':
                        j = i + 1
                        while j < len(mods) and type(mods[j]) is torch.nn.Identity:
                            j += 1
                        if j < len(mods) and type(mods[j]) is NormalLinear and mods[j].in_channels % 8 == 0:
                            if fuse_head and mods[j].weight.mean.shape[0] <= 16 and j == len(mods) - 1:
                                la.__dict__["_fuse_head"] = mods[j]
                            la.out_dtype = torch.bfloat16
                            la.out_x3 = mods[j].weight.mean.shape[0] > 16 or mods[j].in_channels <= 2048
    return fused
```

### bayesianneuralnetworks_amd/nn/dense.py

```python
import math

import torch
from torch.nn import init
from torch.distributions import Normal
from torch.distributions.multivariate_normal import MultivariateNormal

from .. import _mc, ops
from .._rng import default_generator, generator_for
from . import _settings
from .container import BayesianModule
from .core import WeightNormal, WeightMultivariateNormal


class BayesianLinear(BayesianModule):

    def __init__(self, in_features, out_features, bias, weight, prior, bias_prior=None):
        super().__init__(in_features, out_features, prior, bias_prior)
        self.weight = weight(out_features, in_features)
        if bias:
            self.bias = weight(out_features)
        else:
            self.register_parameter('bias', None)
        self.reset_parameters()

    def reset_parameters(self):
        pass


def _init_normal_posterior(layer):
    init.kaiming_uniform_(layer.weight.mean, a=math.sqrt(5))
    init.normal_(layer.weight.scale, -2.0, 0.15)
    if layer.bias is not None:
        fan_in, _ = init._calculate_fan_in_and_fan_out(layer.weight.mean)
        bound = 1 / math.sqrt(fan_in)
        init.uniform_(layer.bias.mean, -bound, bound)
        init.normal_(layer.bias.scale, -2.0, 0.15)


class _NormalSampling:

    compute = None
    activation = None
    out_dtype = None

    def sample(self, nsamples=1, sample0=0):
        epoch = default_generator.next_epoch() if self.weight.mean.is_cuda else None
        gen = generator_for(self._compute_mode())
        self.weight.sample(nsamples, sample0, epoch, gen)
        if self.bias is not None:
            self.bias.sample(nsamples, sample0, epoch, gen)

    def _fresh_keys(self, nsamples, sample0):
        from .._rng import DrawKey
        epoch = default_generator.next_epoch()
        gen = generator_for(self._compute_mode())
        kw = DrawKey(default_generator.seed, self.weight._stream, sample0, nsamples, epoch, gen=gen)
        kb = DrawKey(default_generator.seed, self.bias._stream, sample0, nsamples, epoch, gen=gen) if self.bias is not None else None
        return kw, kb

    def _adopt_keys(self, kw, kb):
        self.weight._key, self.weight._explicit = kw, None
        if self.bias is not None:
            self.bias._key, self.bias._explicit = kb, None

    @property
    def sampled(self):
        return (self.weight.sampled, self.bias.sampled if self.bias is not None else None)

    @sampled.setter
    def sampled(self, value):
        w, b = value
        self.weight.sampled = w
        if self.bias is not None and b is not None:
            self.bias.sampled = b

    def _compute_mode(self):
        return self.compute or _settings.get_compute()

    def _trainable(self):
        ps = [self.weight.mean, self.weight.scale]
        if self.bias is not None:
            ps += [self.bias.mean, self.bias.scale]
        return any(p.requires_grad for p in ps)

    def _mc_plan(self, x, sample):
        ctx = _mc.current()
        if ctx is None or ctx.samples == 1:
            S, s0 = 1, (ctx.sample0 if ctx else 0)
            shared, per = True, x.shape[0]
        else:
            S, s0 = ctx.samples, ctx.sample0
            if x.shape[0] == ctx.base_batch:
                shared, per = True, x.shape[0]
            elif x.shape[0] == ctx.base_batch * S:
                shared, per = False, ctx.base_batch
            else:
                raise RuntimeError("mc_batched: layer input has %d rows, expected %d or %d"
                                   % (x.shape[0], ctx.base_batch, ctx.base_batch * S))
        if sample:
            self.sample(S, s0)
        return S, s0, shared, per

    def _x3_call(self, x, rows):
        if not ops.DENSE_X3_F32:
            return False
        if torch.is_grad_enabled() and (self._trainable() or (torch.is_tensor(x) and x.requires_grad)):
            return False
        if torch.is_tensor(x) and (x.dim() != 2 or x.dtype != torch.float32):
            return False
        x2 = x if isinstance(x, ops.X3Activation) else x
        return ops.x3_eligible(x2, self.weight.mean, rows)

    def _try_fused_head(self, x2, shared, per, S, mode, predrawn, sample_head):
        ctx = _mc.current()
        head = self.__dict__.get("_fuse_head")
        if head is None or ctx is None or not ctx.lazy_head or mode != "bf16" or predrawn is None or torch.is_grad_enabled():
            return None
        hd = getattr(head, "_predrawn", None)
        if hd is None or hd[0] is not ctx or self.out_dtype != torch.bfloat16 or head._compute_mode() != "bf16" or head.activation is not None:
            return None
        K = x2.shape[-1]
        if not ops.dense_head_eligible(per, self.weight.mean.shape[0], predrawn, hd[1]) or predrawn.w.dim() != 3:
            return None
        if x2.dtype == torch.bfloat16:
            pitch = ops.rows_pitch(x2, K)
            xb, ldx, xs = (x2, pitch[0], pitch[1]) if pitch is not None else (x2.contiguous(), K, per * K)
        else:
            xb, ldx, xs = x2.contiguous().to(torch.bfloat16), K, per * K
        head._predrawn = None
        head._adopt_keys(hd[1].key_w, hd[1].key_b)
        predrawn.wait()
        hd[1].wait()
        hp = ops._dense_head_raw(xb, 0 if shared else xs, per, predrawn, K, self.activation == 'relu', hd[1], ldx=ldx)
        hp.head = head
        return hp

    def _keys(self, S):
        kw = self.weight.draw_key
        kb = self.bias.draw_key if self.bias is not None else None
        if kw is None or (self.bias is not None and kb is None):
            return None
        if kw.nsamples != S:
            if S == 1:
                return kw.last_sample(), (kb.last_sample() if kb is not None else None)
            raise RuntimeError("sample=False: the recorded draw has %d MC samples, this call needs %d"
                               % (kw.nsamples, S))
        return kw, kb


class NormalLinear(_NormalSampling, BayesianLinear):

    def __init__(self, in_features, out_features, bias=True, prior=Normal(0, .1)):
        super().__init__(in_features, out_features, bias, WeightNormal, prior)

    def reset_parameters(self):
        _init_normal_posterior(self)
        self.sample()

    def forward(self, x, sample=True):
        if not x.is_cuda:
            if sample:
                self.sample()
            y = torch.nn.functional.linear(x, *self.sampled)
            return torch.relu(y) if self.activation == 'relu' else y
        if isinstance(x, ops.HeadPartials):
            if x.head is not self:
                raise RuntimeError("a fused hidden layer's partial logits reached a layer that is not its head")
            return x
        if x.dim() == 1:
            return self.forward(x.unsqueeze(0), sample).squeeze(0)
        predrawn = None
        pd = getattr(self, "_predrawn", None)
        if pd is not None:
            self._predrawn = None
            if sample and pd[0] is _mc.current():
                predrawn, sample = pd[1], False
                self._adopt_keys(predrawn.key_w, predrawn.key_b)
        S, _, shared, per = self._mc_plan(x, sample)
        keys = self._keys(S)
        mode = self._compute_mode()
        if keys is not None and mode != "bf16" and self._x3_call(x, per):
            K = x.shape[-1]
            ctx = _mc.current()
            xpl = ctx.x_planes if ctx is not None else None
            if xpl is not None and torch.is_tensor(x) and shared and x.data_ptr() == xpl[0].data_ptr() and x.shape == xpl[0].shape:
                x = ops.X3Activation(xpl[1], K)
            x2 = x if isinstance(x, ops.X3Activation) else (x.reshape(-1, K) if shared else x.reshape(S, -1, K))
            pre3 = predrawn if (predrawn is not None and predrawn.w.dim() == 4) else None
            head_pre, head = None, self.__dict__.get("_fuse_head")
            if head is not None and ctx is not None and ctx.lazy_head and pre3 is not None and head.activation is None:
                hd = getattr(head, "_predrawn", None)
                if hd is not None and hd[0] is ctx and head._compute_mode() != "bf16" and \
                        ops.dense_head_x3_eligible(per, self.weight.mean.shape[0], pre3, hd[1]):
                    head._predrawn = None
                    head._adopt_keys(hd[1].key_w, hd[1].key_b)
                    head_pre = hd[1]
            y = ops.linear_sampled_x3(x2, shared, per, self.weight.mean.detach(), self.weight.scale.detach(),
                                      self.bias.mean.detach() if self.bias is not None else None,
                                      self.bias.scale.detach() if self.bias is not None else None,
                                      keys[0], keys[1], relu=self.activation == 'relu',
                                      planes_out=bool(getattr(self, "out_x3", False)),
                                      predrawn=pre3, head_pre=head_pre)
            if isinstance(y, ops.HeadPartials):
                y.head = head
                return y
            if isinstance(y, ops.X3Activation):
                return y
            return y.reshape(S * per, y.shape[-1])
        if isinstance(x, ops.X3Activation):
            x = x.float()
        lead = x.shape[1:-1]
        K = x.shape[-1]
        x2 = x.reshape(-1, K) if shared else x.reshape(S, -1, K)
        if keys is not None:
            odt = torch.bfloat16 if (self.out_dtype == torch.bfloat16 and mode == "bf16") else torch.float32
            hp = self._try_fused_head(x2, shared, per, S, mode, predrawn, sample_head=True)
            if hp is not None:
                return hp
            y = ops.linear_sampled(x2, self.weight.mean, self.weight.scale,
                                   self.bias.mean if self.bias is not None else None,
                                   self.bias.scale if self.bias is not None else None,
                                   keys[0], keys[1], shared, mode, relu=self.activation == 'relu',
                                   out_dtype=odt, predrawn=predrawn if (mode == "bf16" and predrawn is not None and predrawn.w.dim() == 3) else None)
        else:
            w, b = self.sampled
            y = ops.linear_plain(x2.float(), w.unsqueeze(0).expand(S, -1, -1), None if b is None else
                                 b.unsqueeze(0).expand(S, -1), shared, mode)
            if self.activation == 'relu':
                y = torch.relu(y)
        return y.reshape(S * per, *lead, y.shape[-1])


def _flipout_plan(layer, x):
    ctx = _mc.current()
    if ctx is None or not isinstance(x, torch.Tensor) or not x.is_cuda:
        return None
    if x.dim() >= 2 and x.shape[0] == ctx.base_batch:
        return ctx, True
    if x.dim() >= 2 and x.shape[0] == ctx.base_batch * ctx.samples:
        return ctx, False
    raise RuntimeError("mc_batched: %s got an input of shape %s; expected (%d, ...) or (%d, ...) rows (batch %d x %d samples)"
                       % (type(layer).__name__, tuple(x.shape), ctx.base_batch, ctx.base_batch * ctx.samples,
                          ctx.base_batch, ctx.samples))


def _flipout_fresh_key(layer, ctx):
    from .._rng import DrawKey, new_stream_id
    if getattr(layer, "_flip_stream", None) is None:
        layer._flip_stream = new_stream_id()
    return DrawKey(default_generator.seed, layer._flip_stream, ctx.sample0, ctx.samples, default_generator.next_epoch(),
                   gen=generator_for(_settings.get_compute()))


def _flipout_mc_key(layer, ctx, sample):
    if sample:
        layer.flip_key = _flipout_fresh_key(layer, ctx)
        return layer.flip_key
    key = getattr(layer, "flip_key", None)
    if key is None or key.nsamples != ctx.samples:
        raise RuntimeError("sample=False: %s has %s Flipout signs recorded, this MC-batched pass needs %d samples"
                           % (type(layer).__name__, "no" if key is None else "%d samples of" % key.nsamples, ctx.samples))
    return key


class FlipoutNormalLinear(NormalLinear):

    def __init__(self, in_features, out_features, prior=Normal(0, .1)):
        super().__init__(in_features, out_features, False, prior)
        self.flip_key = None
        self._flip_stream = None

    def sample(self, *unused):
        dev = self.weight.device
        self.R = (torch.rand(self.weight.size(0), device=dev) - .5).sign()
        self.S = (torch.rand(self.weight.size(1), device=dev) - .5).sign()

    @property
    def sampled(self):
        return (self.R, self.S)

    def forward(self, x, sample=True):
        plan = _flipout_plan(self, x)
        if plan is not None:
            return self._forward_mc(x, sample, *plan)
        if sample:
            self.sample()
        if not x.is_cuda:
            perturbation = torch.matmul(x * self.S, self.weight.stddev.t()) * self.R
            return torch.nn.functional.linear(x, self.weight.mean, perturbation)
        eps = torch.outer(self.R, self.S)
        w = ops.sample_affine_eps(self.weight.mean, self.weight.scale, eps)
        K = x.shape[-1]
        y = ops.linear_plain(x.reshape(-1, K).float(), w.unsqueeze(0), None, True, self._compute_mode())
        return y.reshape(*x.shape[:-1], y.shape[-1])

    def _forward_mc(self, x, sample, ctx, shared):
        predrawn = None
        pd = getattr(self, "_predrawn", None)
        if pd is not None:
            self._predrawn = None
            if sample and pd[0] is ctx:
                predrawn = pd[1]
                self.flip_key = predrawn.key_w
        key = predrawn.key_w if predrawn is not None else _flipout_mc_key(self, ctx, sample)
        S = key.nsamples
        O, K = self.weight.mean.shape
        x2 = x.reshape(-1, K)
        mode = self._compute_mode()
        if ops.flipout_drawable(self.weight.mean):
            y = ops.linear_flipout_mc(x2, self.weight.mean, self.weight.scale, key, shared, mode,
                                      predrawn if mode == "bf16" else None)
        else:
            sg = ops.flipout_signs(key, 1, O + K, x.device)
            R, Sg = sg[:, :, :O], sg[:, :, O:]
            xs = x2.float().reshape(1 if shared else S, -1, K)
            out = ops.linear_plain(xs.reshape(-1, K), self.weight.mean.unsqueeze(0), None, True, mode).reshape(xs.shape[0], -1, O)
            noise = ops.linear_plain(xs * Sg, self.weight.stddev.unsqueeze(0).expand(S, O, K), None, False, mode)
            y = out + noise * R
        return y.reshape(-1, *x.shape[1:-1], O)


class MultivariateNormalLinear(BayesianLinear):

    def __init__(self, in_features, out_features, bias=True, weight_prior=None, bias_prior=None):
        if not weight_prior:
            weight_prior = MultivariateNormal(torch.zeros(out_features, in_features),
                                              torch.eye(in_features).repeat(out_features, 1, 1))
        if bias and not bias_prior:
            bias_prior = MultivariateNormal(torch.zeros(out_features), torch.eye(out_features))
        super().__init__(in_features, out_features, bias, WeightMultivariateNormal,
                         weight_prior, bias_prior)

    @staticmethod
    def _mask_upper(scale):
        with torch.no_grad():
            upper = torch.triu(torch.ones_like(scale), 1).to(torch.bool)
            scale[upper] = -100

    def reset_parameters(self):
        _init_normal_posterior(self)
        self._mask_upper(self.weight.scale)
        if self.bias is not None:
            self._mask_upper(self.bias.scale)
        self.sample()

    def sample(self):
        self.weight.sample()
        if self.bias is not None:
            self.bias.sample()
            self.sampled = (self.weight.sampled, self.bias.sampled)
        else:
            self.sampled = (self.weight.sampled, None)

    def forward(self, x, sample=True):
        if sample:
            self.sample()
        return torch.nn.functional.linear(x, *self.sampled)


class NormalInverseGaussianLinear(BayesianModule):

    def __init__(self, in_features, out_features, bias=True):
        super().__init__(in_features, out_features, None)
        self.linear = torch.nn.Linear(in_features, 4 * out_features, bias)

    def forward(self, x, sample=False):
        sp = torch.nn.functional.softplus
        gamma, upsilon, alpha, beta = torch.split(self.linear(x), self.out_channels, dim=-1)
        upsilon = 1e-10 + sp(upsilon)
# ... 64 lines not shown
```

### bayesianneuralnetworks_amd/ops.py

```python
import collections
import ctypes
import os
import threading

import torch

from . import _lib
from ._lib import (BnnHipError, Rng, KlTensor, Conv2dShape, ptr, stream_ptr, check, require_cuda_f32,
                   require_cuda_act)
from ._rng import default_generator, DrawKey


def _rng_struct(key, device):
    r = Rng()
    r.seed = key.seed
    r.stream = key.stream
    r.sample0 = key.sample0
    r.epoch_host = key.epoch_host
    r.epoch_dev_delta = key.epoch_dev_delta
    r.epoch_dev = default_generator.epoch_dev(device).data_ptr()
    r.generator = key.gen
    return r


# ... 76 lines not shown
        out = _sample_affine_philox_raw(mu.detach(), rho.detach(), key)
        ctx.save_for_backward(rho)
        ctx.key = key
        return out

    @staticmethod
    def backward(ctx, g):
        (rho,) = ctx.saved_tensors
        g_mu, g_rho = _sample_affine_bwd_raw(g, rho, rho.numel(), ctx.key.nsamples, key=ctx.key)
        return g_mu, g_rho, None


def sample_affine_eps(mu, rho, eps):
    return _SampleAffineEps.apply(mu.contiguous(), rho.contiguous(), eps.contiguous())


def sample_affine_philox(mu, rho, key):
    return _SampleAffinePhilox.apply(mu.contiguous(), rho.contiguous(), key)


def _pad64(k):
    return (k + 63) // 64 * 64


def dense_eligible(mu_w):
    return mu_w.dim() == 2 and mu_w.shape[1] % 8 == 0 and mu_w.data_ptr() % 16 == 0


class Predrawn:
    __slots__ = ("w", "b", "key_w", "key_b", "ready")

    def __init__(self, w, b, key_w, key_b, ready=None):
        self.w, self.b, self.key_w, self.key_b, self.ready = w, b, key_w, key_b, ready

    def wait(self):
        if self.ready is not None:
            torch.cuda.current_stream(self.w.device).wait_stream(self.ready)
            self.ready = None


_side_streams = {}


def side_stream(device):
    key = (device.type, device.index)
    st = _side_streams.get(key)
    if st is None:
        st = torch.cuda.Stream(device)
        _side_streams[key] = st
    return st


def draw_layers(layers, nsamples, kl=None, stream=None, x3=False, split=None):
    _tls.last_split = None
    out = []
    lib = _lib.load()
    dev = layers[0][0].device
    cur = torch.cuda.current_stream(dev)
    if stream is not None:
        stream.wait_stream(cur)
    launch_stream = stream if stream is not None else cur
    sp = _lib.stream_ptr(dev)
    sp.value = launch_stream.cuda_stream
    step = 4 if split is None else 3
    for i0 in range(0, len(layers), step):
        group = layers[i0:i0 + step]
        arr = (_lib.DrawTensor * (2 * len(group) + 1))()
        n = 0
        keep = []
        if split is not None and i0 == 0 and x3:
            require_cuda_f32(split, "x")
            Ms, Ks = split.shape
            lds_ = _pad64(Ks)
            planes = torch.empty((3, 1, Ms, lds_), dtype=torch.bfloat16, device=dev)
            t = arr[n]
            t.mu, t.rho, t.rows, t.cols = split.data_ptr(), split.data_ptr(), Ms, Ks
            t.out, t.ld, t.out_sample_stride, t.out_dtype = planes.data_ptr(), lds_, Ms * lds_, _lib.BF16X3
            t.kind, t.taps = 3, 0
            n += 1
            _tls.last_split = planes
            keep.append(split)
        for spec in group:
            mu_w, rho_w, mu_b, rho_b, key_w, key_b = spec[:6]
            taps = spec[6] if len(spec) > 6 else 0
            kind = spec[7] if len(spec) > 7 else 0
            require_cuda_f32(mu_w, "weight.mean")
            require_cuda_f32(rho_w, "weight.scale")
            N, K = mu_w.shape
            kp = _pad64(K)
            w = torch.empty(((3, nsamples, N, kp) if x3 else (nsamples, N, kp)), dtype=torch.bfloat16, device=dev)
            t = arr[n]
            t.mu, t.rho, t.rows, t.cols = mu_w.data_ptr(), rho_w.data_ptr(), N, K
            t.out, t.ld, t.out_sample_stride, t.out_dtype = w.data_ptr(), kp, N * kp, (_lib.BF16X3 if x3 else _lib.BF16)
            t.taps, t.kind = taps, kind
            t.rng = _rng_struct(key_w, dev)
            n += 1
            b = None
            if mu_b is not None:
                require_cuda_f32(mu_b, "bias.mean")
                require_cuda_f32(rho_b, "bias.scale")
                b = torch.empty((nsamples, N), dtype=torch.float32, device=dev)
                t = arr[n]
                t.mu, t.rho, t.rows, t.cols = mu_b.data_ptr(), rho_b.data_ptr(), 1, N
                t.out, t.ld, t.out_sample_stride, t.out_dtype = b.data_ptr(), N, N, _lib.F32
                t.taps = 0
                t.rng = _rng_struct(key_b, dev)
                n += 1
            keep.append((mu_w, rho_w, mu_b, rho_b))
            out.append(Predrawn(w, b, key_w, key_b, ready=stream))
        carried = False
        if kl is not None and not kl.launched and i0 == 0 and kl.out.device == dev:
            rc = lib.bnn_draw_multi(arr, n, nsamples, kl.arr, kl.T, ptr(kl.ws), sp)
            if rc == 0:
                kl.launched = carried = True
            elif rc != _lib.E_UNSUPPORTED:
                check(rc, "bnn_draw_multi")
        if not carried:
            check(lib.bnn_draw_multi(arr, n, nsamples, None, 0, None, sp), "bnn_draw_multi")
    return out


def rows_pitch(t, K):
    if t.dtype != torch.bfloat16 or t.dim() not in (2, 3) or t.shape[-1] != K or t.stride(-1) != 1 or t.data_ptr() % 16 != 0:
        return None
    M = t.shape[-2]
    ld = t.stride(-2) if M > 1 else K
    if ld < K or ld % 8 != 0:
        return None
    if t.dim() == 2 or t.shape[0] == 1:
        return ld, M * ld
    xs = t.stride(0)
    if xs % 8 != 0 or xs < (M - 1) * ld + K:
        return None
    return ld, xs


def rows_regular(t, K):
    return rows_pitch(t, K) is not None


def _dense_raw(x2, x_sample_stride, M, pre, K, relu, out_dtype, ldx=None, pad_rows=False):
    S, N, kp = pre.w.shape
    ldx = K if ldx is None else ldx
    ldy = _pad64(N) if (pad_rows and out_dtype == torch.bfloat16) else N
    ybuf = torch.empty((S, M, ldy), dtype=out_dtype, device=x2.device)
    flags = (_lib.FLAG_RELU if relu else 0) | (_lib.FLAG_Y_BF16 if out_dtype == torch.bfloat16 else 0)
    check(_lib.load().bnn_dense_forward(ptr(x2), x_sample_stride, ldx, ptr(pre.w), N * kp, kp,
                                         ptr(pre.b), N if pre.b is not None else 0, ptr(ybuf), M * ldy, ldy, M, N, K, S, flags,
                                         stream_ptr(x2.device)), "bnn_dense_forward")
    return ybuf if ldy == N else ybuf[:, :, :N]


class HeadPartials:
    __slots__ = ("p", "head")

    def __init__(self, p, head=None):
        self.p, self.head = p, head

    @property
    def shape(self):
        return torch.Size((self.p.shape[1] * self.p.shape[2], self.p.shape[3]))

    @property
    def is_cuda(self):
        return True

    @property
    def device(self):
        return self.p.device

    def dim(self):
        return 2

    def logits(self):
        parts, S, M, Nh = self.p.shape
        out = torch.empty((S, M, Nh), dtype=torch.float32, device=self.p.device)
        n = S * M * Nh
        check(_lib.load().bnn_mc_sum(ptr(self.p), n, parts, n, 1.0, ptr(out), 0, None, 0, stream_ptr(self.p.device)), "bnn_mc_sum")
        return out


def dense_head_eligible(M, N, pre, pre_head):
    return (pre is not None and pre_head is not None and pre.w.dim() == 3 and pre_head.w.dim() == 3 and N > 16 and N % 8 == 0 and
            pre_head.w.shape[1] <= 16 and pre_head.w.shape[2] >= N and pre.w.shape[0] == pre_head.w.shape[0] and M > 0)


def _dense_head_raw(x2, x_sample_stride, M, pre, K, relu, pre_head, ldx=None):
    S, N, kp = pre.w.shape
    _, Nh, kph = pre_head.w.shape
    lib = _lib.load()
    parts = lib.bnn_dense_head_parts(M, N, S)
    P = torch.empty((parts, S, M, Nh), dtype=torch.float32, device=x2.device)
    ldx = K if ldx is None else ldx
    check(lib.bnn_dense_forward_head(ptr(x2), x_sample_stride, ldx, ptr(pre.w), N * kp, kp, ptr(pre.b), N if pre.b is not None else 0,
                                     ptr(pre_head.w), Nh * kph, kph, ptr(pre_head.b), Nh if pre_head.b is not None else 0, Nh,
                                     ptr(P), M, N, K, S, _lib.FLAG_RELU if relu else 0, stream_ptr(x2.device)), "bnn_dense_forward_head")
    return HeadPartials(P)


def dense_head_x3_eligible(M, N, pre, pre_head):
    return (pre is not None and pre_head is not None and pre.w.dim() == 4 and pre_head.w.dim() == 4 and N > 80 and N % 8 == 0 and
            (N % 80 == 0 or N < 128) and pre_head.w.shape[2] <= 16 and pre_head.w.shape[3] >= N and pre.w.shape[1] == pre_head.w.shape[1] and M > 0)


def _dense_head_raw_x3(xp, shared, M, pre, K, relu, pre_head):
    _, S, N, kp = pre.w.shape
    _, _, Nh, kph = pre_head.w.shape
    ldx = xp.shape[3]
    lib = _lib.load()
    parts = lib.bnn_dense_head_parts(M, N, S)
    P = torch.empty((parts, S, M, Nh), dtype=torch.float32, device=xp.device)
    check(lib.bnn_dense_forward_x3_head(ptr(xp), xp.shape[1] * M * ldx, 0 if shared else M * ldx, ldx,
                                        ptr(pre.w), S * N * kp, N * kp, kp, ptr(pre.b), N if pre.b is not None else 0,
                                        ptr(pre_head.w), S * Nh * kph, Nh * kph, kph, ptr(pre_head.b), Nh if pre_head.b is not None else 0, Nh,
                                        ptr(P), M, N, K, S, _lib.FLAG_RELU if relu else 0, stream_ptr(xp.device)), "bnn_dense_forward_x3_head")
    return HeadPartials(P)


class X3Activation:
    __slots__ = ("planes", "cols")

    def __init__(self, planes, cols):
        self.planes, self.cols = planes, cols

    @property
    def shape(self):
        return torch.Size((self.planes.shape[1] * self.planes.shape[2], self.cols))

    @property
    def is_cuda(self):
        return self.planes.is_cuda

    @property
    def device(self):
        return self.planes.device

    def dim(self):
        return 2

    def float(self):
        p = self.planes[..., :self.cols].float()
        return (p[0] + p[1] + p[2]).reshape(-1, self.cols)


def split_x3(x2):
    require_cuda_f32(x2, "x")
    M, K = x2.shape
    ld = _pad64(K)
    out = torch.empty((3, 1, M, ld), dtype=torch.bfloat16, device=x2.device)
    check(_lib.load().bnn_split_bf16x3(ptr(x2), M, K, x2.stride(0) if M > 1 else K, ptr(out), ld, M * ld, stream_ptr(x2.device)),
          "bnn_split_bf16x3")
    return out


def x3_eligible(x2, mu_w, M):
    N, K = mu_w.shape
    if not (dense_eligible(mu_w) and M >= 64 and (N > 16 or K <= 2048)):
        return False
    if isinstance(x2, X3Activation):
        return True
    return x2.dtype == torch.float32 and x2.dim() == 2 and x2.stride(-1) == 1 and x2.stride(0) % 4 == 0 and x2.data_ptr() % 16 == 0


def _dense_raw_x3(xp, shared, M, pre, K, relu, planes_out):
    _, S, N, kp = pre.w.shape
    ldx = xp.shape[3]
    xs = 0 if shared else M * ldx
    if planes_out:
        ldy = _pad64(N)
        y = torch.empty((3, S, M, ldy), dtype=torch.bfloat16, device=xp.device)
        yps = S * M * ldy
    else:
        ldy = N
        y = torch.empty((S, M, N), dtype=torch.float32, device=xp.device)
        yps = 0
    flags = (_lib.FLAG_RELU if relu else 0) | (_lib.FLAG_Y_BF16 if planes_out else 0)
    check(_lib.load().bnn_dense_forward_x3(ptr(xp), xp.shape[1] * M * ldx, xs, ldx, ptr(pre.w), S * N * kp, N * kp, kp,
                                            ptr(pre.b), N if pre.b is not None else 0, ptr(y), yps, M * ldy, ldy, M, N, K, S, flags,
                                            stream_ptr(xp.device)), "bnn_dense_forward_x3")
    return X3Activation(y, N) if planes_out else y


def linear_sampled_x3(x2, shared, M, mu_w, rho_w, mu_b, rho_b, key_w, key_b, relu=False, planes_out=False, predrawn=None, head_pre=None):
    S = key_w.nsamples
    N, K = mu_w.shape
    pre = predrawn
    if pre is None:
        pre = draw_layers([(mu_w, rho_w, mu_b, rho_b, key_w, key_b)], S, kl=_tls.kl_carry, x3=True)[0]
        if _tls.kl_carry is not None and _tls.kl_carry.launched:
            _tls.kl_carry = None
    pre.wait()
    if isinstance(x2, X3Activation):
        xp = x2.planes
        if xp.shape[1] not in (1, S) or xp.shape[2] != M or x2.cols != K:
            raise BnnHipError("linear: three-plane activation of shape %s does not fit (S = %d, M = %d, K = %d)" % (tuple(xp.shape), S, M, K))
        shared = xp.shape[1] == 1
    else:
        xp = split_x3(x2.reshape(-1, K))
        if not shared:
            xp = xp.view(3, S, M, xp.shape[3])
    if head_pre is not None:
        head_pre.wait()
        return _dense_head_raw_x3(xp, shared, M, pre, K, relu, head_pre)
    return _dense_raw_x3(xp, shared, M, pre, K, relu, planes_out)


def _linear_sampled_raw(x2, x_sample_stride, M, mu_w, rho_w, mu_b, rho_b, key_w, key_b, compute, relu=False,
                        out_dtype=torch.float32, predrawn=None, pad_rows=False):
    N, K = mu_w.shape
    S = key_w.nsamples
    _lib.ensure_workspace(x2.device)
    if compute == _lib.COMPUTE_BF16 and DRAW_ONCE_BF16 and dense_eligible(mu_w) and M > 0:
        pre = predrawn
        if pre is None:
            pre = draw_layers([(mu_w, rho_w, mu_b, rho_b, key_w, key_b)], S, kl=_tls.kl_carry)[0]
            if _tls.kl_carry is not None and _tls.kl_carry.launched:
                _tls.kl_carry = None
        pre.wait()
        pitch = rows_pitch(x2, K) if x2.dtype == torch.bfloat16 else None
        if pitch is not None:
            ldx, xs = pitch
            return _dense_raw(x2, 0 if x_sample_stride == 0 else xs, M, pre, K, relu, out_dtype, ldx=ldx, pad_rows=pad_rows)
        xb = x2.contiguous().to(torch.bfloat16)
        return _dense_raw(xb, x_sample_stride, M, pre, K, relu, out_dtype, pad_rows=pad_rows)
    x2 = x2.contiguous()
    y = torch.empty((S, M, N), dtype=out_dtype, device=x2.device)
    rw = _rng_struct(key_w, x2.device)
    rb = _rng_struct(key_b, x2.device) if mu_b is not None else None
    flags = (_lib.FLAG_RELU if relu else 0) | (_lib.FLAG_X_BF16 if x2.dtype == torch.bfloat16 else 0) | \
            (_lib.FLAG_Y_BF16 if out_dtype == torch.bfloat16 else 0)
    if (M >= DRAW_ONCE_MIN_ROWS and N > 16 and K % 8 == 0 and mu_w.data_ptr() % 16 == 0 and rho_w.data_ptr() % 16 == 0):
        w = _sample_affine_philox_raw(mu_w.reshape(-1), rho_w.reshape(-1), key_w)
        b = _sample_affine_philox_raw(mu_b, rho_b, key_b) if mu_b is not None else None
        check(_lib.load().bnn_linear_forward(ptr(x2), x_sample_stride, K, ptr(w), N * K, ptr(b), N, ptr(y), M * N, N, M, N, K, S,
                                              compute, flags, stream_ptr(x2.device)), "bnn_linear_forward")
        return y
    h = _tls.kl_carry
    if h is not None and N <= 16 and not h.launched and h.out.device == x2.device:
        check(_lib.load().bnn_linear_forward_sampled_kl(
            ptr(x2), x_sample_stride, K, ptr(mu_w), ptr(rho_w), ptr(mu_b), ptr(rho_b),
            ptr(y), M * N, N, M, N, K, S, ctypes.byref(rw), ctypes.byref(rb) if rb is not None else None,
            compute, flags, h.arr, h.T, ptr(h.ws), stream_ptr(x2.device)), "bnn_linear_forward_sampled_kl")
        h.launched = True
        _tls.kl_carry = None
        return y
    check(_lib.load().bnn_linear_forward_sampled(
        ptr(x2), x_sample_stride, K, ptr(mu_w), ptr(rho_w), ptr(mu_b), ptr(rho_b),
        ptr(y), M * N, N, M, N, K, S, ctypes.byref(rw), ctypes.byref(rb) if rb is not None else None,
        compute, flags, stream_ptr(x2.device)), "bnn_linear_forward_sampled")
# ... 1250 lines not shown
```

### include/bnn_hip.h

```cpp
#ifndef BNN_HIP_H
#define BNN_HIP_H

#include <stdint.h>

#ifdef __cplusplus
extern "C" {
#endif

#define BNN_ABI_VERSION 2

enum {
    BNN_OK = 0,
    BNN_E_NULL = -1,
    BNN_E_SHAPE = -2,
    BNN_E_DTYPE = -3,
    BNN_E_ALIGN = -4,
    BNN_E_RANGE = -5,
    BNN_E_UNSUPPORTED = -6,
    BNN_E_DEVICE = -7
};

enum { BNN_F32 = 0, BNN_BF16 = 1,
       BNN_BF16X3 = 2  };

enum {
    BNN_COMPUTE_F32 = 0,
    BNN_COMPUTE_BF16 = 1
};

enum { BNN_GEN_PHILOX10_U24 = 0, BNN_GEN_PHILOX7_U16 = 1 };

typedef struct bnn_rng {
    uint64_t seed;
    uint32_t stream;
    uint32_t sample0;
    uint32_t epoch_host;
    int32_t epoch_dev_delta;
    const uint32_t *epoch_dev;
    uint32_t generator;
    uint32_t reserved;
} bnn_rng_t;

typedef struct bnn_kl_tensor {
    const float *mu;
    const float *rho;
    int64_t n;
    float prior_mu;
    float prior_sigma;
} bnn_kl_tensor_t;

int bnn_abi_version(void);
const char *bnn_arch(void);
const char *bnn_last_error(void);
uint64_t bnn_launch_count(void);

int bnn_set_workspace(int device, void *ptr, int64_t bytes);
int bnn_check_device(int device, void *stream);

int bnn_sample_affine_eps(const float *mu, const float *rho, const float *eps,
                          void *out, int64_t n, int out_dtype, void *stream);
int bnn_sample_affine_philox(const float *mu, const float *rho, void *out, int64_t n,
                             int nsamples, int64_t out_sample_stride, int out_dtype,
                             const bnn_rng_t *rng, void *stream);
int bnn_eps_philox(float *out, int64_t n, int nsamples, int64_t out_sample_stride,
                   const bnn_rng_t *rng, void *stream);
int bnn_sigma(const float *rho, float *out, int64_t n, void *stream);

int bnn_sample_affine_bwd(const float *g_w, int64_t g_w_sample_stride, const float *rho,
                          const float *eps, int64_t eps_sample_stride, const bnn_rng_t *rng,
                          int64_t n, int nsamples, float *g_mu, float *g_rho, int accumulate,
                          void *stream);

int bnn_rng_advance(uint32_t *epoch_dev, uint32_t inc, void *stream);

int64_t bnn_kl_workspace_bytes(int ntensors);
int bnn_kl_forward(const bnn_kl_tensor_t *tensors, int ntensors, float n_batches,
                   float *out, void *workspace, void *stream);
int bnn_kl_forward_partial(const bnn_kl_tensor_t *tensors, int ntensors, void *workspace, void *stream);
int bnn_kl_backward(const bnn_kl_tensor_t *tensors, int ntensors, float n_batches,
                    const float *upstream, float *const *g_mu, float *const *g_rho,
                    int accumulate, void *stream);

enum {
    BNN_FLAG_RELU = 1,
    BNN_FLAG_X_BF16 = 2,
    BNN_FLAG_Y_BF16 = 4
};
int bnn_linear_forward_sampled(const void *x, int64_t x_sample_stride, int64_t ldx,
                               const float *mu_w, const float *rho_w,
                               const float *mu_b, const float *rho_b,
                               void *y, int64_t y_sample_stride, int64_t ldy,
                               int64_t M, int64_t N, int64_t K, int nsamples,
                               const bnn_rng_t *rng_w, const bnn_rng_t *rng_b,
                               int compute, int flags, void *stream);
int bnn_linear_forward_sampled_kl(const void *x, int64_t x_sample_stride, int64_t ldx,
                                  const float *mu_w, const float *rho_w, const float *mu_b,
                                  const float *rho_b, void *y, int64_t y_sample_stride, int64_t ldy,
                                  int64_t M, int64_t N, int64_t K, int nsamples, const bnn_rng_t *rng_w,
                                  const bnn_rng_t *rng_b, int compute, int flags,
                                  const bnn_kl_tensor_t *tensors, int ntensors, void *kl_workspace, void *stream);
enum { BNN_DRAW_FLIPOUT = 16 };
typedef struct bnn_draw_tensor {
    const float *mu;
    const float *rho;
    int64_t rows, cols;
    void *out;
    int64_t ld;
    int64_t out_sample_stride;
    int out_dtype;
    int kind;
    int taps;
    bnn_rng_t rng;
} bnn_draw_tensor_t;
int bnn_draw_multi(const bnn_draw_tensor_t *tensors, int ntensors, int nsamples,
                   const bnn_kl_tensor_t *kl_tensors, int kl_ntensors, void *kl_workspace, void *stream);
int bnn_dense_forward(const void *x, int64_t x_sample_stride, int64_t ldx,
                      const void *w, int64_t w_sample_stride, int64_t ldw,
                      const float *b, int64_t b_sample_stride,
                      void *y, int64_t y_sample_stride, int64_t ldy,
                      int64_t M, int64_t N, int64_t K, int nsamples, int flags, void *stream);
int bnn_dense_forward_dropout(const void *x, int64_t x_sample_stride, int64_t ldx,
                              const void *w, int64_t w_sample_stride, int64_t ldw,
                              const float *b, int64_t b_sample_stride,
                              void *y, int64_t y_sample_stride, int64_t ldy,
                              int64_t M, int64_t N, int64_t K, int nsamples, int flags, float p, const bnn_rng_t *rng, void *stream);
int bnn_dense_head_parts(int64_t M, int64_t N, int nsamples);
int bnn_dense_forward_head(const void *x, int64_t x_sample_stride, int64_t ldx,
                           const void *w, int64_t w_sample_stride, int64_t ldw,
                           const float *b, int64_t b_sample_stride,
                           const void *w_head, int64_t wh_sample_stride, int64_t ldwh,
                           const float *b_head, int64_t bh_sample_stride, int64_t n_head,
                           float *partials, int64_t M, int64_t N, int64_t K, int nsamples, int flags, void *stream);
int bnn_dense_forward_x3_head(const void *x, int64_t x_plane_stride, int64_t x_sample_stride, int64_t ldx,
                              const void *w, int64_t w_plane_stride, int64_t w_sample_stride, int64_t ldw,
                              const float *b, int64_t b_sample_stride,
                              const void *w_head, int64_t wh_plane_stride, int64_t wh_sample_stride, int64_t ldwh,
                              const float *b_head, int64_t bh_sample_stride, int64_t n_head,
                              float *partials, int64_t M, int64_t N, int64_t K, int nsamples, int flags, void *stream);
int bnn_dense_forward_x3(const void *x, int64_t x_plane_stride, int64_t x_sample_stride, int64_t ldx,
                         const void *w, int64_t w_plane_stride, int64_t w_sample_stride, int64_t ldw,
                         const float *b, int64_t b_sample_stride,
                         void *y, int64_t y_plane_stride, int64_t y_sample_stride, int64_t ldy,
                         int64_t M, int64_t N, int64_t K, int nsamples, int flags, void *stream);
int bnn_split_bf16x3(const float *x, int64_t rows, int64_t cols, int64_t ldx, void *out, int64_t ld_out, int64_t plane_stride,
                     void *stream);
int bnn_transpose_bf16(const void *in, int64_t in_batch_stride, int64_t ld_in, void *out, int64_t out_batch_stride, int64_t ld_out,
                       int64_t rows, int64_t cols, int batch, void *stream);

int bnn_linear_forward(const float *x, int64_t x_sample_stride, int64_t ldx,
                       const float *w, int64_t w_sample_stride,
                       const float *b, int64_t b_sample_stride,
                       float *y, int64_t y_sample_stride, int64_t ldy,
                       int64_t M, int64_t N, int64_t K, int nsamples,
                       int compute, int flags, void *stream);

int bnn_linear_backward_input_sampled(const void *gy, int64_t gy_sample_stride, int64_t ldgy,
                                      const float *mu_w, const float *rho_w,
                                      void *gx, int64_t gx_sample_stride, int64_t ldgx,
                                      int64_t M, int64_t N, int64_t K, int nsamples,
                                      const bnn_rng_t *rng_w, int compute, int flags, void *stream);
int bnn_linear_backward_input(const void *gy, int64_t gy_sample_stride, int64_t ldgy,
                              const float *w, int64_t w_sample_stride,
                              void *gx, int64_t gx_sample_stride, int64_t ldgx,
                              int64_t M, int64_t N, int64_t K, int nsamples, int flags, void *stream);
typedef struct bnn_kl_fuse {
    const float *upstream;
    const float *mu_w;
    const float *mu_b;
    float scale_w, prior_mu_w, prior_sigma_w;
    float scale_b, prior_mu_b, prior_sigma_b;
} bnn_kl_fuse_t;
int bnn_linear_backward_weight_sampled(const void *x, int64_t x_sample_stride, int64_t ldx,
                                       const void *gy, int64_t gy_sample_stride, int64_t ldgy,
                                       const float *rho_w, float *g_mu, float *g_rho,
                                       const float *rho_b, float *g_mu_b, float *g_rho_b,
                                       int64_t M, int64_t N, int64_t K, int nsamples,
                                       const bnn_rng_t *rng_w, const bnn_rng_t *rng_b,
                                       const bnn_kl_fuse_t *kl,
                                       int compute, int flags, int accumulate, void *stream);
int bnn_linear_backward_narrow_sampled(const void *x, int64_t x_sample_stride, int64_t ldx,
                                       const float *gy, int64_t gy_sample_stride, int64_t ldgy,
                                       const float *mu_w, const float *rho_w,
                                       void *gx, int64_t gx_sample_stride, int64_t ldgx,
                                       float *g_mu, float *g_rho,
                                       const float *rho_b, float *g_mu_b, float *g_rho_b,
                                       int64_t M, int64_t N, int64_t K, int nsamples,
                                       const bnn_rng_t *rng_w, const bnn_rng_t *rng_b,
                                       const bnn_kl_fuse_t *kl, int flags, int accumulate, void *stream);
int bnn_linear_backward_weight(const void *x, int64_t x_sample_stride, int64_t ldx,
                               const void *gy, int64_t gy_sample_stride, int64_t ldgy,
                               float *gw, int64_t gw_sample_stride,
                               int64_t M, int64_t N, int64_t K, int nsamples,
                               int compute, int flags, int accumulate, void *stream);
int bnn_colsum(const void *gy, int64_t gy_sample_stride, int64_t ldgy, float *out,
               int64_t M, int64_t N, int nsamples, int flags, void *stream);
int bnn_relu_backward(const void *g, const void *y, void *out, int64_t n, int flags, void *stream);

typedef struct bnn_conv2d_shape {
    int32_t B, C, H, W;
    int32_t O, KH, KW;
    int32_t stride_h, stride_w, pad_h, pad_w, dil_h, dil_w, groups;
} bnn_conv2d_shape_t;
int64_t bnn_conv2d_workspace_bytes(const bnn_conv2d_shape_t *shape, int x_samples, int compute);
int bnn_conv2d_forward_sampled(const float *x, int64_t x_sample_stride,
                               const float *mu_w, const float *rho_w,
                               const float *mu_b, const float *rho_b,
                               float *y, int64_t y_sample_stride,
                               const bnn_conv2d_shape_t *shape, int nsamples,
                               const bnn_rng_t *rng_w, const bnn_rng_t *rng_b,
                               int compute, int flags,
                               void *workspace, int64_t workspace_bytes, void *stream);
int bnn_conv2d_forward(const float *x, int64_t x_sample_stride,
                       const float *w, int64_t w_sample_stride,
                       const float *b, int64_t b_sample_stride,
                       float *y, int64_t y_sample_stride,
                       const bnn_conv2d_shape_t *shape, int nsamples,
                       int compute, int flags,
                       void *workspace, int64_t workspace_bytes, void *stream);

int bnn_conv2d_dense_forward(const float *x, int64_t x_sample_stride,
                             const void *w, int64_t w_sample_stride, int64_t ldw,
                             const float *b, int64_t b_sample_stride,
                             float *y, int64_t y_sample_stride,
                             const bnn_conv2d_shape_t *shape, int nsamples, int flags, void *stream);

int bnn_conv2d_dense_forward_x3(const float *x, int64_t x_sample_stride,
                                const void *w, int64_t w_plane_stride, int64_t w_sample_stride, int64_t ldw,
                                const float *b, int64_t b_sample_stride,
                                float *y, int64_t y_sample_stride,
                                const bnn_conv2d_shape_t *sh, int nsamples, int flags, void *stream);
int bnn_conv2d_flipout_forward(const float *x, const void *w, int64_t ldw, const float *sign_in, const float *sign_out,
                               float *y, const bnn_conv2d_shape_t *shape, int flags, void *stream);
int bnn_conv2d_flipout_forward_x3(const float *x, const void *w, int64_t w_plane_stride, int64_t ldw, const float *sign_in,
                                  const float *sign_out, float *y, const bnn_conv2d_shape_t *sh, int flags, void *stream);

int bnn_conv2d_flipout_forward_mc(const float *x, int64_t x_sample_stride, const void *w, int64_t ldw, float *y,
                                  int64_t y_sample_stride, const bnn_conv2d_shape_t *shape, int nsamples, const bnn_rng_t *rng,
                                  int flags, void *stream);

int bnn_conv2d_im2col(const float *x, int64_t x_sample_stride, const bnn_conv2d_shape_t *shape,
                      int x_samples, void *panel, int out_bf16, void *stream);
int bnn_conv2d_col2im(const float *gpanel, const bnn_conv2d_shape_t *shape, int nsamples,
                      int shared_x, float *gx, void *stream);
int bnn_nchw_to_rows(const float *y, int64_t images, int channels, int pixels, void *rows,
                     int out_bf16, void *stream);

int bnn_diag_sampler(float *out, int blocks, int iters, int stage, void *stream);
int bnn_diag_astream(const float *x, int S, int M, int K, int rows_per_wg, int ntn, int pattern,
                     int nwaves, float *out, void *stream);

typedef struct bnn_adam_tensor {
    float *p;
    const float *g;
    float *m;
    float *v;
    int64_t n;
} bnn_adam_tensor_t;
int bnn_adam_step(const bnn_adam_tensor_t *tensors, int ntensors, float lr, float beta1, float beta2,
                  float eps, float weight_decay, float *step, void *stream);
int bnn_adam_step_advance(const bnn_adam_tensor_t *tensors, int ntensors, float lr, float beta1, float beta2,
                          float eps, float weight_decay, float *step, uint32_t *advance_epoch,
                          uint32_t advance_inc, void *stream);
int64_t bnn_xent_workspace_bytes(int64_t rows);
int bnn_softmax_xent(const float *logits, const int64_t *target, int64_t rows, int classes,
                     float *loss, float *g_logits, void *workspace, void *stream);

int bnn_prune_score(const float *mu, const float *rho, float *out, int64_t n, void *stream);

int bnn_mc_dropout(const void *x, int64_t x_sample_stride, void *y, int64_t y_sample_stride, int64_t rows, int64_t features,
                   int nsamples, float p, int dtype, const bnn_rng_t *rng, void *stream);
int bnn_mc_dropout_backward(const float *gy, int64_t gy_sample_stride, float *gx, int64_t gx_sample_stride, int64_t rows,
                            int64_t features, int nsamples, float p, int sum_samples, const bnn_rng_t *rng, void *stream);

int bnn_flipout_signs(float *out, int64_t out_sample_stride, int64_t rows, int64_t width, int nsamples, const bnn_rng_t *rng,
                      void *stream);
int bnn_flipout_weight_backward(const float *g_w, int64_t g_w_sample_stride, const float *rho, float *g_mu, float *g_rho,
                                int64_t O, int64_t K, int nsamples, const bnn_rng_t *rng, void *stream);

int bnn_mc_sum(const float *y, int64_t y_sample_stride, int nsamples, int64_t n,
               float scale, float *out, int accumulate, uint32_t *advance_epoch,
               uint32_t advance_inc, void *stream);

int bnn_mc_sum_kl(const float *y, int64_t y_sample_stride, int nsamples, int64_t n,
                  float scale, float *out, int accumulate, uint32_t *advance_epoch,
                  uint32_t advance_inc, const bnn_kl_tensor_t *tensors, int ntensors,
// ... 15 lines not shown
```

Baseline: 199,100.

## Fuse both hidden BNN layers and head into one persistent chained kernel

```diff
diff --git a/bayesianneuralnetworks_amd/_lib.py b/bayesianneuralnetworks_amd/_lib.py
--- a/bayesianneuralnetworks_amd/_lib.py
+++ b/bayesianneuralnetworks_amd/_lib.py
@@ -103,6 +103,10 @@
     "bnn_flipout_weight_backward": (_int, [_p, _i64, _p, _p, _p, _i64, _i64, _int, _rngp, _p]),
     "bnn_mc_dropout_backward": (_int, [_p, _i64, _p, _i64, _i64, _i64, _int, _f, _int, _rngp, _p]),
     "bnn_dense_head_parts": (_int, [_i64, _i64, _int]),
+    "bnn_dense_chain_eligible": (_int, [_i64, _i64, _i64, _i64, _int]),
+    "bnn_dense_chain_workspace_bytes": (_i64, [_i64, _int]),
+    "bnn_dense_forward_chain": (_int, [_p, _i64, _i64, _p, _i64, _i64, _p, _i64, _p, _i64, _i64, _p, _i64, _i64, _p, _i64,
+                                       _p, _i64, _i64, _p, _i64, _i64, _p, _i64, _i64, _i64, _i64, _int, _int, _p, _i64, _p]),
     "bnn_dense_forward_head": (_int, [_p, _i64, _i64, _p, _i64, _i64, _p, _i64, _p, _i64, _i64, _p, _i64, _i64,
                                       _p, _i64, _i64, _i64, _int, _int, _p]),
     "bnn_dense_forward_x3_head": (_int, [_p, _i64, _i64, _i64, _p, _i64, _i64, _i64, _p, _i64, _p, _i64, _i64, _i64,
diff --git a/bayesianneuralnetworks_amd/csrc/bnn_dense.hip b/bayesianneuralnetworks_amd/csrc/bnn_dense.hip
--- a/bayesianneuralnetworks_amd/csrc/bnn_dense.hip
+++ b/bayesianneuralnetworks_amd/csrc/bnn_dense.hip
@@ -3,6 +3,7 @@
 
 #include "bnn_device.hpp"
 #include "bnn_dma.hpp"
+#include "bnn_gemm_params.hpp"
 #include "bnn_kl_body.hpp"
 
 namespace bnn {
@@ -1481,6 +1482,417 @@
             *reinterpret_cast<uint4 *>(dst + (int64_t)(c0 + c) * ld_out + r0 + rc) = *reinterpret_cast<const uint4 *>(&T[c * PITCH + rc]);
     }
 }
+
+struct ChainParams {
+    DenseParams l[2];
+    unsigned *ws;
+    unsigned *dev_err;
+    int32_t ntm, ntn1, ntn2;
+    int32_t per1, per2;
+    int32_t groups;
+};
+constexpr int kChainLine = 32;
+constexpr int kChainWs = 9;
+constexpr uint32_t kChainSpins = 1u << 20;
+
+typedef uint32_t u32x4 __attribute__((ext_vector_type(4)));
+__device__ __forceinline__ void st_sc1_b128(void *q, uint4 v)
+{
+    const u32x4 w = {v.x, v.y, v.z, v.w};
+    asm volatile("global_store_dwordx4 %0, %1, off sc1" :: "v"(q), "v"(w) : "memory");
+}
+__device__ __forceinline__ void st_sc1_b16(void *q, uint32_t v)
+{
+    asm volatile("global_store_short %0, %1, off sc1" :: "v"(q), "v"(v) : "memory");
+}
+
+__device__ __forceinline__ const void *uniform_ptr(const void *q)
+{
+    const uint64_t v = reinterpret_cast<uint64_t>(q);
+    const uint32_t lo = __builtin_amdgcn_readfirstlane((uint32_t)v), hi = __builtin_amdgcn_readfirstlane((uint32_t)(v >> 32));
+    return reinterpret_cast<const void *>(((uint64_t)hi << 32) | lo);
+}
+
+template <bool RELU2>
+__global__ __launch_bounds__(512) void k_dense_chain(const ChainParams P)
+{
+    constexpr int TM = 4, TN = 5, NWM = 2, NWN = 2, ST = 4, NWV = 4, MPR = 2;
+    constexpr int WM = 16 * TM, WN = 16 * TN, BM = NWM * WM, BN = NWN * WN;
+    constexpr int A_PIECES = BM / 8 / NWV, B_PIECES = BN / 8 / NWV;
+    static_assert((BN / 8) % NWV == 0, "B pieces divide evenly over the loaders");
+    constexpr int A_STAGE = BM * 128, B_STAGE = BN * 128, STAGE = A_STAGE + B_STAGE;
+    constexpr int PITCH = WN * 2 + 16;
+    constexpr int EPI = 16 * PITCH;
+    __shared__ __attribute__((aligned(16))) char lds[ST * STAGE + NWV * EPI];
+    __shared__ int tix[4];
+
+    const int tid = threadIdx.x, lane = tid & 63;
+    const int wave = __builtin_amdgcn_readfirstlane(tid >> 6);
+    const int grp = (int)blockIdx.x % P.groups;
+    const int total = P.per1 + P.per2;
+    unsigned *const ready = P.ws + kChainWs * kChainLine;
+    auto claim = [&]() -> int {
+        const unsigned q = __hip_atomic_fetch_add(P.ws + grp * kChainLine, 1u, __ATOMIC_RELAXED, __HIP_MEMORY_SCOPE_AGENT);
+        return q < (unsigned)total ? (int)q : -1;
+    };
+    struct Tile { int layer, s, mt, panel, nk; };
+    auto decode = [&](int q) {
+        Tile t;
+        t.layer = q >= P.per1;
+        const int r = t.layer ? q - P.per1 : q;
+        const int ntn = t.layer ? P.ntn2 : P.ntn1;
+        const int per_s = P.ntm * ntn;
+        const int j = r / per_s, u = r - j * per_s;
+        t.s = grp + P.groups * j;
+        t.mt = u / ntn;
+        t.panel = u - t.mt * ntn;
+        t.nk = (P.l[t.layer].K + 63) >> 6;
+        return t;
+    };
+    auto read_tix = [&](int ord) {
+        return __builtin_amdgcn_readfirstlane(__hip_atomic_load(&tix[ord & 3], __ATOMIC_RELAXED, __HIP_MEMORY_SCOPE_WORKGROUP));
+    };
+    if (wave == NWV && lane == 0) tix[0] = claim();
+    asm volatile("s_waitcnt lgkmcnt(0)" ::: "memory");
+    __builtin_amdgcn_s_barrier();
+    asm volatile("" ::: "memory");
+
+    if (wave >= NWV) {
+        const int lw = wave - NWV;
+        const uint32_t ring = __builtin_amdgcn_readfirstlane(lds_addr_of(lds));
+        const int prow = lane >> 3;
+        const int schunk = (lane & 7) ^ prow;
+        bool gave_up = false;
+        int ord_i = 0, k_i = 0, nk_i = 0;
+        bool rdy_i = true, end_i = false;
+        const char *ab = nullptr, *wb = nullptr;
+        const unsigned *rdy_ctr = nullptr;
+        uint32_t a_off[A_PIECES], b_off[B_PIECES], a_colmax = 0;
+        auto set_tile = [&](int q) {
+            const Tile t = decode(q);
+            const DenseParams &p = P.l[t.layer];
+            ab = reinterpret_cast<const char *>(p.A + (int64_t)t.s * p.a_sample_stride);
+            wb = reinterpret_cast<const char *>(p.W + (int64_t)t.s * p.w_sample_stride);
+            const int m0 = t.mt * BM, n0 = t.panel * BN;
+#pragma unroll
+            for (int j = 0; j < A_PIECES; ++j) {
+                int m = m0 + (lw + NWV * j) * 8 + prow;
+                m = m < p.M ? m : p.M - 1;
+                a_off[j] = (uint32_t)((int64_t)m * p.lda * 2);
+            }
+#pragma unroll
+            for (int j = 0; j < B_PIECES; ++j) {
+                int n = n0 + (lw + NWV * j) * 8 + prow;
+                n = n < p.N ? n : p.N - 1;
+                b_off[j] = (uint32_t)((int64_t)n * p.ldw * 2) + 16u * (uint32_t)schunk;
+            }
+            a_colmax = (uint32_t)(p.K * 2 - 16);
+            nk_i = t.nk;
+            rdy_ctr = t.layer ? ready + (t.s * P.ntm + t.mt) * kChainLine : nullptr;
+            rdy_i = t.layer == 0;
+        };
+        uint32_t a_dst[A_PIECES], b_dst[B_PIECES];
+#pragma unroll
+        for (int j = 0; j < A_PIECES; ++j) {
+            const int r0 = (lw + NWV * j) * 8;
+            a_dst[j] = (uint32_t)((r0 / WM) * (ST * WM * 128) + (r0 % WM) * 128);
+        }
+#pragma unroll
+        for (int j = 0; j < B_PIECES; ++j) {
+            const int r0 = (lw + NWV * j) * 8;
+            b_dst[j] = (uint32_t)(ST * A_STAGE + (r0 / WN) * (ST * WN * 128) + (r0 % WN) * 128);
+        }
+        const unsigned target = 4u * (unsigned)P.ntn1;
+        auto poll = [&](bool blocking) -> bool {
+            for (uint32_t spin = 0;; ++spin) {
+                unsigned v = 0;
+                if (lane == 0) v = __hip_atomic_load(rdy_ctr, __ATOMIC_RELAXED, __HIP_MEMORY_SCOPE_AGENT);
+                v = __builtin_amdgcn_readfirstlane(v);
+                if (v >= target || gave_up) break;
+                if (!blocking) return false;
+                if (spin >= kChainSpins) {
+                    gave_up = true;
+                    if (P.dev_err && lane == 0) __hip_atomic_fetch_or(P.dev_err, kDevErrChainTimeout, __ATOMIC_RELAXED, __HIP_MEMORY_SCOPE_AGENT);
+                    break;
+                }
+                __builtin_amdgcn_s_sleep(8);
+            }
+            __builtin_amdgcn_fence(__ATOMIC_ACQUIRE, "agent");
+            return true;
+        };
+        int issued = 0;
+        auto issue = [&]() {
+            const int stage = issued % ST;
+            const uint32_t colA0 = (uint32_t)(k_i * 128 + 16 * schunk);
+            const uint32_t colA = colA0 < a_colmax ? colA0 : a_colmax;
+            const uint32_t colB = (uint32_t)(k_i * 128);
+            const uint32_t sa = ring + (uint32_t)(stage * (WM * 128)), sb = ring + (uint32_t)(stage * (WN * 128));
+            const char *abu = reinterpret_cast<const char *>(uniform_ptr(ab)), *wbu = reinterpret_cast<const char *>(uniform_ptr(wb));
+#pragma unroll
+            for (int j = 0; j < A_PIECES; ++j) dma_piece(abu, a_off[j] + colA, __builtin_amdgcn_readfirstlane(sa + a_dst[j]));
+#pragma unroll
+            for (int j = 0; j < B_PIECES; ++j) dma_piece(wbu, b_off[j] + colB, __builtin_amdgcn_readfirstlane(sb + b_dst[j]));
+        };
+        auto try_issue = [&](int limit, bool blocking) {
+            while (issued < limit && !end_i) {
+                if (k_i == nk_i) {
+                    ++ord_i;
+                    const int q = read_tix(ord_i);
+                    if (q < 0) { end_i = true; break; }
+                    set_tile(q);
+                    k_i = 0;
+                }
+                if (!rdy_i) {
+                    rdy_i = poll(blocking);
+                    if (!rdy_i) break;
+                }
+                issue();
+                if (lw == 0 && k_i == nk_i - 1) {
+                    if (lane == 0) tix[(ord_i + 1) & 3] = claim();
+                    asm volatile("s_waitcnt lgkmcnt(0)" ::: "memory");
+                }
+                ++k_i;
+                ++issued;
+            }
+        };
+        int q = read_tix(0);
+        if (q >= 0) {
+            set_tile(q);
+            if (!rdy_i) rdy_i = poll(true);
+            try_issue(ST - 1, true);
+            int g = 0, k_c = 0, nk_c = nk_i, ord_c = 0;
+            while (true) {
+                if (issued <= g) try_issue(g + ST - 1, true);
+                const int ahead = issued - 1 - g;
+                if (ahead >= 2) asm volatile("s_waitcnt vmcnt(%0)" :: "n"(2 * (A_PIECES + B_PIECES)) : "memory");
+                else if (ahead == 1) asm volatile("s_waitcnt vmcnt(%0)" :: "n"(A_PIECES + B_PIECES) : "memory");
+                else asm volatile("s_waitcnt vmcnt(0)" ::: "memory");
+                __builtin_amdgcn_s_barrier();
+                ++g;
+                if (++k_c == nk_c) {
+                    q = read_tix(++ord_c);
+                    if (q < 0) break;
+                    nk_c = decode(q).nk;
+                    k_c = 0;
+                }
+                try_issue(g + ST - 1, false);
+            }
+        }
+    } else {
+        const int fi = lane & 15, fq = lane >> 4;
+        const int wm = wave / NWN, wn = wave % NWN;
+        const char *a_rows = lds + wm * (ST * WM * 128);
+        const char *b_rows = lds + ST * A_STAGE + wn * (ST * WN * 128);
+        char *const T = lds + ST * STAGE + wave * EPI;
+        const int fbase0 = fi * 128 + (((0 + fq) ^ (fi & 7)) << 4);
+        const int fbase1 = fi * 128 + (((4 + fq) ^ (fi & 7)) << 4);
+        f32x4 acc[TM][TN];
+        uint4 fa[2][TM], fb[2][TN];
+        auto rd = [&](auto buf_c, uint32_t stage, auto h_c) {
+            constexpr int buf = decltype(buf_c)::value, h = decltype(h_c)::value;
+            const char *As = a_rows + (stage * (uint32_t)(WM * 128) + (uint32_t)(h ? fbase1 : fbase0));
+            const char *Bs = b_rows + (stage * (uint32_t)(WN * 128) + (uint32_t)(h ? fbase1 : fbase0));
+#pragma unroll
+            for (int b = 0; b < TN; ++b) fb[buf][b] = *reinterpret_cast<const uint4 *>(Bs + b * 2048);
+#pragma unroll
+            for (int a = 0; a < TM; ++a) fa[buf][a] = *reinterpret_cast<const uint4 *>(As + a * 2048);
+        };
+        auto mm = [&](auto buf_c) {
+            constexpr int buf = decltype(buf_c)::value;
+#pragma unroll
+            for (int a = 0; a < TM; ++a)
+#pragma unroll
+                for (int b = 0; b < TN; ++b)
+                    acc[a][b] = __builtin_amdgcn_mfma_f32_16x16x32_bf16(__builtin_bit_cast(bf16x8, fb[buf][b]),
+                                                                        __builtin_bit_cast(bf16x8, fa[buf][a]), acc[a][b], 0, 0, 0);
+        };
+        using I0 = std::integral_constant<int, 0>;
+        using I1 = std::integral_constant<int, 1>;
+        auto interleave = [&]() {
+            constexpr int NI = (TM * TN) / MPR < TM + TN ? (TM * TN) / MPR : TM + TN;
+#pragma unroll
+            for (int i = 0; i < NI; ++i) {
+                __builtin_amdgcn_sched_group_barrier(0x008, MPR, 0);
+                __builtin_amdgcn_sched_group_barrier(0x100, 1, 0);
+            }
+            if constexpr (TM + TN > NI) __builtin_amdgcn_sched_group_barrier(0x100, TM + TN - NI, 0);
+            if constexpr (TM * TN > MPR * NI) __builtin_amdgcn_sched_group_barrier(0x008, TM * TN - MPR * NI, 0);
+        };
+        auto first_half = [&](uint32_t stage) {
+            rd(I1{}, stage, I1{});
+            mm(I0{});
+            interleave();
+            __builtin_amdgcn_sched_barrier(0);
+        };
+        auto second_half = [&](uint32_t next) {
+            asm volatile("s_waitcnt lgkmcnt(0)" ::: "memory");
+            __builtin_amdgcn_s_barrier();
+            asm volatile("" ::: "memory");
+            rd(I0{}, next, I0{});
+            mm(I1{});
+            interleave();
+            __builtin_amdgcn_sched_barrier(0);
+        };
+        uint32_t stage = 0;
+        for (int ord = 0;; ++ord) {
+            const int q = read_tix(ord);
+            if (q < 0) break;
+            const Tile t = decode(q);
+            const DenseParams &p = P.l[t.layer];
+            const int s = t.s, panel = t.panel;
+            const int mw = t.mt * BM + wm * WM, nw = panel * BN + wn * WN;
+            const int nk = t.nk;
+            if (nw >= p.N || mw >= p.M) {
+                for (int kt = 0; kt < nk; ++kt) __builtin_amdgcn_s_barrier();
+                stage = (stage + (uint32_t)nk) % ST;
+                if (t.layer) {
+                    float *Pp = p.P + ((int64_t)(panel * NWN + wn) * p.S + s) * (int64_t)p.M * p.Nh;
+                    for (int i = lane; i < WM * p.Nh; i += 64) {
+                        const int m = mw + i / p.Nh;
+                        if (m < p.M) Pp[(int64_t)m * p.Nh + (i % p.Nh)] = 0.f;
+                    }
+                } else {
+                    if (lane == 0) __hip_atomic_fetch_add(ready + (s * P.ntm + t.mt) * kChainLine, 1u, __ATOMIC_RELAXED, __HIP_MEMORY_SCOPE_AGENT);
+                }
+                continue;
+            }
+            const float *bias = p.bias ? p.bias + (int64_t)s * p.bias_sample_stride : nullptr;
+            float bv[TN][4];
+#pragma unroll
+            for (int b = 0; b < TN; ++b)
+#pragma unroll
+                for (int r = 0; r < 4; ++r) {
+                    const int n = nw + b * 16 + fq * 4 + r;
+                    bv[b][r] = (bias && n < p.N) ? bias[n] : 0.f;
+                }
+#pragma unroll
+            for (int a = 0; a < TM; ++a)
+#pragma unroll
+                for (int b = 0; b < TN; ++b) acc[a][b] = f32x4{0.f, 0.f, 0.f, 0.f};
+            __builtin_amdgcn_s_setprio(1);
+            __builtin_amdgcn_s_barrier();
+            asm volatile("" ::: "memory");
+            rd(I0{}, stage, I0{});
+            for (int kt = 0; kt + 1 < nk; ++kt) {
+                const uint32_t next = stage + 1 == (uint32_t)ST ? 0u : stage + 1;
+                first_half(stage);
+                second_half(next);
+                stage = next;
+            }
+            first_half(stage);
+            mm(I1{});
+            __builtin_amdgcn_sched_barrier(0);
+            __builtin_amdgcn_s_setprio(0);
+            asm volatile("s_waitcnt lgkmcnt(0)" ::: "memory");
+            stage = stage + 1 == (uint32_t)ST ? 0u : stage + 1;
+            const bool relu = t.layer == 0 || RELU2;
+            auto vals = [&](int a, int b, float (&v)[4]) {
+#pragma unroll
+                for (int r = 0; r < 4; ++r) {
+                    v[r] = acc[a][b][r] + bv[b][r];
+                    if (relu) v[r] = fmaxf(v[r], 0.f);
+                }
+            };
+            if (t.layer == 0) {
+                const bool wide = nw + WN <= p.N && mw + WM <= p.M && (p.ldy * 2) % 16 == 0 && (nw * 2) % 16 == 0 &&
+                                  ((reinterpret_cast<uintptr_t>(p.Y) + (int64_t)s * p.y_sample_stride * 2) & 15u) == 0;
+                char *Y8 = reinterpret_cast<char *>(p.Y) + ((int64_t)s * p.y_sample_stride + (int64_t)mw * p.ldy + nw) * 2;
+                if (wide) {
+                    constexpr int cpr = WN * 2 / 16;
+#pragma unroll
+                    for (int a = 0; a < TM; ++a) {
+#pragma unroll
+                        for (int b = 0; b < TN; ++b) {
+                            float v[4];
+                            vals(a, b, v);
+                            *reinterpret_cast<uint2 *>(T + fi * PITCH + (b * 16 + fq * 4) * 2) = make_uint2(pack_bf16x2(v[0], v[1]), pack_bf16x2(v[2], v[3]));
+                        }
+                        __builtin_amdgcn_fence(__ATOMIC_RELEASE, "workgroup");
+                        __builtin_amdgcn_wave_barrier();
+                        for (int c = lane; c < 16 * cpr; c += 64) {
+                            const int row = c / cpr, cc = c - row * cpr;
+                            st_sc1_b128(Y8 + (int64_t)(a * 16 + row) * p.ldy * 2 + cc * 16, *reinterpret_cast<const uint4 *>(T + row * PITCH + cc * 16));
+                        }
+                        __builtin_amdgcn_fence(__ATOMIC_RELEASE, "workgroup");
+                        __builtin_amdgcn_wave_barrier();
+                    }
+                } else {
+                    uint16_t *Yh = reinterpret_cast<uint16_t *>(p.Y) + (int64_t)s * p.y_sample_stride;
+#pragma unroll
+                    for (int a = 0; a < TM; ++a) {
+                        const int m = mw + a * 16 + fi;
+                        if (m >= p.M) continue;
+#pragma unroll
+                        for (int b = 0; b < TN; ++b) {
+                            float v[4];
+                            vals(a, b, v);
+#pragma unroll
+                            for (int r = 0; r < 4; ++r) {
+                                const int n = nw + b * 16 + fq * 4 + r;
+                                if (n < p.N) st_sc1_b16(Yh + (int64_t)m * p.ldy + n, f2bf(v[r]));
+                            }
+                        }
+                    }
+                }
+                asm volatile("s_waitcnt vmcnt(0)" ::: "memory");
+                if (lane == 0) __hip_atomic_fetch_add(ready + (s * P.ntm + t.mt) * kChainLine, 1u, __ATOMIC_RELAXED, __HIP_MEMORY_SCOPE_AGENT);
+            } else {
+                const int Nh = p.Nh;
+                const int hrow = fi < Nh ? fi : Nh - 1;
+                const uint16_t *wh = p.Wh + (int64_t)s * p.wh_sample_stride + (int64_t)hrow * p.ldwh;
+                constexpr int NC = (WN + 31) / 32;
+                uint4 bf[NC];
+#pragma unroll
+                for (int c = 0; c < NC; ++c) {
+                    const int kcol = 32 * c + 8 * fq;
+                    const int n = nw + kcol;
+                    bf[c] = make_uint4(0u, 0u, 0u, 0u);
+                    if (kcol < WN && fi < Nh && n + 8 <= (int)p.ldwh) bf[c] = *reinterpret_cast<const uint4 *>(wh + n);
+                }
+                const int part = panel * NWN + wn;
+                float hb = 0.f;
+                if (part == 0 && p.bias_h && fi < Nh) hb = p.bias_h[(int64_t)s * p.bias_h_sample_stride + fi];
+                float *Pp = p.P + ((int64_t)part * p.S + s) * (int64_t)p.M * Nh;
+#pragma unroll
+                for (int a = 0; a < TM; ++a) {
+#pragma unroll
+                    for (int b = 0; b < TN; ++b) {
+                        float v[4];
+                        vals(a, b, v);
+                        *reinterpret_cast<uint2 *>(T + fi * PITCH + (b * 16 + fq * 4) * 2) = make_uint2(pack_bf16x2(v[0], v[1]), pack_bf16x2(v[2], v[3]));
+                    }
+                    __builtin_amdgcn_fence(__ATOMIC_RELEASE, "workgroup");
+                    __builtin_amdgcn_wave_barrier();
+                    f32x4 hacc = f32x4{0.f, 0.f, 0.f, 0.f};
+#pragma unroll
+                    for (int c = 0; c < NC; ++c) {
+                        const int kcol = 32 * c + 8 * fq;
+                        uint4 af = make_uint4(0u, 0u, 0u, 0u);
+                        if (kcol < WN) af = *reinterpret_cast<const uint4 *>(T + fi * PITCH + kcol * 2);
+                        hacc = __builtin_amdgcn_mfma_f32_16x16x32_bf16(__builtin_bit_cast(bf16x8, af), __builtin_bit_cast(bf16x8, bf[c]), hacc, 0, 0, 0);
+                    }
+                    __builtin_amdgcn_fence(__ATOMIC_RELEASE, "workgroup");
+                    __builtin_amdgcn_wave_barrier();
+#pragma unroll
+                    for (int r = 0; r < 4; ++r) {
+                        const int m = mw + a * 16 + fq * 4 + r;
+                        if (m < p.M && fi < Nh) Pp[(int64_t)m * Nh + fi] = hacc[r] + hb;
+                    }
+                }
+            }
+        }
+    }
+    asm volatile("s_waitcnt vmcnt(0)" ::: "memory");
+    __builtin_amdgcn_s_barrier();
+    if (wave == 0) {
+        unsigned last = 0;
+        if (lane == 0) last = __hip_atomic_fetch_add(P.ws + 8 * kChainLine, 1u, __ATOMIC_RELAXED, __HIP_MEMORY_SCOPE_AGENT) == gridDim.x - 1 ? 1u : 0u;
+        if (__builtin_amdgcn_readfirstlane(last)) {
+            const int n = kChainWs + P.l[0].S * P.ntm;
+            for (int i = lane; i < n; i += 64) __hip_atomic_store(P.ws + i * kChainLine, 0u, __ATOMIC_RELAXED, __HIP_MEMORY_SCOPE_AGENT);
+        }
+    }
+}
 }
 
 struct HeadArgs {
@@ -1513,14 +1925,12 @@
     return tile;
 }
 
-static int dense_launch(const char *who, const void *x, int64_t x_plane_stride, int64_t x_sample_stride, int64_t ldx,
-                        const void *w, int64_t w_plane_stride, int64_t w_sample_stride, int64_t ldw,
-                        const float *b, int64_t b_sample_stride,
-                        void *y, int64_t y_plane_stride, int64_t y_sample_stride, int64_t ldy,
-                        int64_t M, int64_t N, int64_t K, int nsamples, int flags, bool x3, void *stream, const HeadArgs *head = nullptr,
-                        const DropArgs *drop = nullptr)
-{
-    if (M == 0 && N >= 1 && K >= 1 && nsamples >= 1) return BNN_OK;
+static int dense_check(const char *who, const void *x, int64_t x_plane_stride, int64_t x_sample_stride, int64_t ldx,
+                       const void *w, int64_t w_plane_stride, int64_t w_sample_stride, int64_t ldw,
+                       const float *b, int64_t b_sample_stride,
+                       void *y, int64_t y_plane_stride, int64_t y_sample_stride, int64_t ldy,
+                       int64_t M, int64_t N, int64_t K, int nsamples, int flags, bool x3, const HeadArgs *head, DenseParams &p)
+{
     if (head) { y = head->partials; ldy = N; }
     if (!x || !w || !y) { set_error("%s: NULL pointer", who); return BNN_E_NULL; }
     if (M < 0 || N < 1 || K < 1 || nsamples < 1 || ldx < K || ldy < N) { set_error("%s: bad extent", who); return BNN_E_SHAPE; }
@@ -1534,7 +1944,6 @@
     if (M * ldx * 2 >= ((int64_t)1 << 32) || N * ldw * 2 >= ((int64_t)1 << 32)) { set_error("%s: one sample's operand exceeds 4 GiB", who); return BNN_E_RANGE; }
     const bool ybf = (flags & BNN_FLAG_Y_BF16) != 0;
     if (reinterpret_cast<uintptr_t>(y) & (ybf ? 1u : 3u)) { set_error("%s: misaligned output", who); return BNN_E_ALIGN; }
-    DenseParams p{};
     p.A = reinterpret_cast<const uint16_t *>(x); p.a_sample_stride = x_sample_stride; p.lda = ldx;
     p.W = reinterpret_cast<const uint16_t *>(w); p.w_sample_stride = w_sample_stride; p.ldw = ldw;
     p.bias = b; p.bias_sample_stride = b_sample_stride;
@@ -1567,6 +1976,24 @@
         p.P = head->partials; p.Nh = (int32_t)head->nh;
         p.wh_plane_stride = head->wh_plane_stride;
     }
+    return BNN_OK;
+}
+
+static int dense_launch(const char *who, const void *x, int64_t x_plane_stride, int64_t x_sample_stride, int64_t ldx,
+                        const void *w, int64_t w_plane_stride, int64_t w_sample_stride, int64_t ldw,
+                        const float *b, int64_t b_sample_stride,
+                        void *y, int64_t y_plane_stride, int64_t y_sample_stride, int64_t ldy,
+                        int64_t M, int64_t N, int64_t K, int nsamples, int flags, bool x3, void *stream, const HeadArgs *head = nullptr,
+                        const DropArgs *drop = nullptr)
+{
+    if (M == 0 && N >= 1 && K >= 1 && nsamples >= 1) return BNN_OK;
+    DenseParams p{};
+    {
+        const int rc = dense_check(who, x, x_plane_stride, x_sample_stride, ldx, w, w_plane_stride, w_sample_stride, ldw, b, b_sample_stride,
+                                   y, y_plane_stride, y_sample_stride, ldy, M, N, K, nsamples, flags, x3, head, p);
+        if (rc != BNN_OK) return rc;
+    }
+    const bool ybf = (flags & BNN_FLAG_Y_BF16) != 0;
     hipStream_t st = (hipStream_t)stream;
     const int full_samples = nsamples;
     if (drop) {
@@ -1818,6 +2245,71 @@
                         b, b_sample_stride, y, y_plane_stride, y_sample_stride, ldy, M, N, K, nsamples, flags, true, stream);
 }
 
+static bool chain_on()
+{
+    const char *e = getenv("BNN_DENSE_CHAIN");
+    return e && e[0] == '1';
+}
+
+int bnn_dense_chain_eligible(int64_t M, int64_t N1, int64_t K1, int64_t N2, int nsamples)
+{
+    return chain_on() && M >= 1 && nsamples >= 8 && nsamples % 8 == 0 && K1 > 192 && N1 > 192 && N2 > 16 &&
+           dense_pick_tile(M, N1, nsamples) == 1 && dense_pick_tile(M, N2, nsamples) == 1 ? 1 : 0;
+}
+
+int64_t bnn_dense_chain_workspace_bytes(int64_t M, int nsamples)
+{
+    if (M < 1 || nsamples < 1) return 0;
+    return (kChainWs + (int64_t)nsamples * ((M + 127) / 128)) * kChainLine * 4;
+}
+
+int bnn_dense_forward_chain(const void *x, int64_t x_sample_stride, int64_t ldx,
+                            const void *w1, int64_t w1_sample_stride, int64_t ldw1, const float *b1, int64_t b1_sample_stride,
+                            void *h1, int64_t h1_sample_stride, int64_t ldh,
+                            const void *w2, int64_t w2_sample_stride, int64_t ldw2, const float *b2, int64_t b2_sample_stride,
+                            const void *w_head, int64_t wh_sample_stride, int64_t ldwh, const float *b_head, int64_t bh_sample_stride,
+                            int64_t n_head, float *partials, int64_t M, int64_t N1, int64_t K1, int64_t N2, int nsamples, int flags,
+                            void *workspace, int64_t workspace_bytes, void *stream)
+{
+    const char *who = "bnn_dense_forward_chain";
+    ChainParams P{};
+    int rc = dense_check(who, x, 0, x_sample_stride, ldx, w1, 0, w1_sample_stride, ldw1, b1, b1_sample_stride, h1, 0, h1_sample_stride, ldh,
+                         M, N1, K1, nsamples, BNN_FLAG_RELU | BNN_FLAG_Y_BF16, false, nullptr, P.l[0]);
+    if (rc != BNN_OK) return rc;
+    HeadArgs h{w_head, 0, wh_sample_stride, ldwh, b_head, bh_sample_stride, partials, n_head};
+    rc = dense_check(who, h1, 0, h1_sample_stride, ldh, w2, 0, w2_sample_stride, ldw2, b2, b2_sample_stride, nullptr, 0, 0, N2,
+                     M, N2, N1, nsamples, flags | BNN_FLAG_Y_BF16, false, &h, P.l[1]);
+    if (rc != BNN_OK) return rc;
+    if (!bnn_dense_chain_eligible(M, N1, K1, N2, nsamples)) {
+        set_error("%s: not a chain shape (S %% 8 == 0, both layers on the 128 x 160 tile, K1 and N1 > 192) or BNN_DENSE_CHAIN is not 1", who);
+        return BNN_E_UNSUPPORTED;
+    }
+    if (!al16(h1) || h1_sample_stride % 8 != 0 || h1_sample_stride < M * ldh) { set_error("%s: h1 needs 16-B aligned, non-overlapping samples", who); return BNN_E_SHAPE; }
+    if (!workspace || (reinterpret_cast<uintptr_t>(workspace) & 15u) || workspace_bytes < bnn_dense_chain_workspace_bytes(M, nsamples)) {
+        set_error("%s: workspace of bnn_dense_chain_workspace_bytes(M, nsamples) zeroed bytes needed", who);
+        return BNN_E_SHAPE;
+    }
+    P.ws = reinterpret_cast<unsigned *>(workspace);
+    P.dev_err = device_error_word();
+    P.ntm = (int32_t)((M + 127) / 128);
+    P.ntn1 = (int32_t)((N1 + 159) / 160);
+    P.ntn2 = (int32_t)((N2 + 159) / 160);
+    P.groups = 8;
+    P.per1 = nsamples / 8 * P.ntm * P.ntn1;
+    P.per2 = nsamples / 8 * P.ntm * P.ntn2;
+    for (int i = 0; i < 2; ++i) { P.l[i].ntm = P.ntm; P.l[i].ntn = i ? P.ntn2 : P.ntn1; }
+    int grid = 256;
+    if (const char *e = getenv("BNN_DENSE_CHAIN_GRID")) {
+        const int g = atoi(e);
+        if (g >= 8 && g % 8 == 0 && g <= 4096) grid = g;
+    }
+    const int64_t tickets = (int64_t)(P.per1 + P.per2) * 8;
+    if (grid > tickets) grid = (int)((tickets + 7) / 8 * 8);
+    if (flags & BNN_FLAG_RELU) hipLaunchKernelGGL(k_dense_chain<true>, dim3((unsigned)grid), dim3(512), 0, (hipStream_t)stream, P);
+    else hipLaunchKernelGGL(k_dense_chain<false>, dim3((unsigned)grid), dim3(512), 0, (hipStream_t)stream, P);
+    return check_launch(who);
+}
+
 int bnn_split_bf16x3(const float *x, int64_t rows, int64_t cols, int64_t ldx, void *out, int64_t ld_out, int64_t plane_stride, void *stream)
 {
     const char *who = "bnn_split_bf16x3";
diff --git a/bayesianneuralnetworks_amd/csrc/bnn_gemm.hip b/bayesianneuralnetworks_amd/csrc/bnn_gemm.hip
--- a/bayesianneuralnetworks_amd/csrc/bnn_gemm.hip
+++ b/bayesianneuralnetworks_amd/csrc/bnn_gemm.hip
@@ -353,6 +353,13 @@
     p.dev_err = reinterpret_cast<unsigned *>(g_ws[dev]);
     p.ws_slabs = reinterpret_cast<float *>(reinterpret_cast<char *>(g_ws[dev]) + kTicketBytes);
     p.ws_slab_bytes = g_ws_bytes[dev] - kTicketBytes;
+}
+
+unsigned *device_error_word()
+{
+    int dev = 0;
+    if (hipGetDevice(&dev) != hipSuccess || dev < 0 || dev >= 64 || !g_ws[dev] || g_ws_bytes[dev] <= kTicketBytes) return nullptr;
+    return reinterpret_cast<unsigned *>(g_ws[dev]);
 }
 
 static inline bool al16(const void *q) { return (reinterpret_cast<uintptr_t>(q) & 15u) == 0; }
diff --git a/bayesianneuralnetworks_amd/csrc/bnn_gemm_params.hpp b/bayesianneuralnetworks_amd/csrc/bnn_gemm_params.hpp
--- a/bayesianneuralnetworks_amd/csrc/bnn_gemm_params.hpp
+++ b/bayesianneuralnetworks_amd/csrc/bnn_gemm_params.hpp
@@ -9,6 +9,7 @@
 
 constexpr int kFlagStoreNCHW = 1 << 16;
 constexpr unsigned kDevErrHandoffTimeout = 1u;
+constexpr unsigned kDevErrChainTimeout = 2u;
 constexpr int kComputeBf16x3 = 2;
 
 struct GemmParams {
@@ -47,5 +48,6 @@
 int dispatch_linear_v2(GemmParams &p, bool sampled, int compute, hipStream_t st, const char *who);
 int dispatch_linear_dgrad(GemmParams &p, int compute, hipStream_t st, const char *who);
 void fill_workspace(GemmParams &p);
+unsigned *device_error_word();
 
 }
diff --git a/bayesianneuralnetworks_amd/nn/_settings.py b/bayesianneuralnetworks_amd/nn/_settings.py
--- a/bayesianneuralnetworks_amd/nn/_settings.py
+++ b/bayesianneuralnetworks_amd/nn/_settings.py
@@ -42,4 +42,11 @@
                                 la.__dict__["_fuse_head"] = mods[j]
                             la.out_dtype = torch.bfloat16
                             la.out_x3 = mods[j].weight.mean.shape[0] > 16 or mods[j].in_channels <= 2048
+                for i, la in enumerate(mods):
+                    if type(la) is NormalLinear and la.out_dtype == torch.bfloat16:
+                        j = i + 1
+                        while j < len(mods) and type(mods[j]) is torch.nn.Identity:
+                            j += 1
+                        if j < len(mods) and "_fuse_head" in mods[j].__dict__:
+                            la.__dict__["_fuse_chain"] = mods[j]
     return fused
diff --git a/bayesianneuralnetworks_amd/nn/dense.py b/bayesianneuralnetworks_amd/nn/dense.py
--- a/bayesianneuralnetworks_amd/nn/dense.py
+++ b/bayesianneuralnetworks_amd/nn/dense.py
@@ -135,6 +135,34 @@
         hp.head = head
         return hp
 
+    def _try_chain(self, x2, shared, per, S, mode, predrawn):
+        ctx = _mc.current()
+        l2 = self.__dict__.get("_fuse_chain")
+        if l2 is None or ctx is None or not ctx.lazy_head or mode != "bf16" or predrawn is None or torch.is_grad_enabled():
+            return None
+        head = l2.__dict__.get("_fuse_head")
+        if head is None or self.out_dtype != torch.bfloat16 or self.activation != 'relu' or l2.out_dtype != torch.bfloat16 or \
+                l2._compute_mode() != "bf16" or head._compute_mode() != "bf16" or head.activation is not None:
+            return None
+        p2, hd = getattr(l2, "_predrawn", None), getattr(head, "_predrawn", None)
+        if p2 is None or hd is None or p2[0] is not ctx or hd[0] is not ctx:
+            return None
+        K = x2.shape[-1]
+        if not ops.dense_chain_eligible(per, K, predrawn, p2[1], hd[1]):
+            return None
+        if x2.dtype == torch.bfloat16:
+            pitch = ops.rows_pitch(x2, K)
+            xb, ldx, xs = (x2, pitch[0], pitch[1]) if pitch is not None else (x2.contiguous(), K, per * K)
+        else:
+            xb, ldx, xs = x2.contiguous().to(torch.bfloat16), K, per * K
+        for m, d in ((l2, p2[1]), (head, hd[1])):
+            m._predrawn = None
+            m._adopt_keys(d.key_w, d.key_b)
+        predrawn.wait()
+        p2[1].wait()
+        hd[1].wait()
+        return ops._dense_chain_raw(xb, 0 if shared else xs, per, predrawn, K, p2[1], l2.activation == 'relu', hd[1], ldx=ldx)._via(l2, head)
+
     def _keys(self, S):
         kw = self.weight.draw_key
         kb = self.bias.draw_key if self.bias is not None else None
@@ -164,7 +192,7 @@
             y = torch.nn.functional.linear(x, *self.sampled)
             return torch.relu(y) if self.activation == 'relu' else y
         if isinstance(x, ops.HeadPartials):
-            if x.head is not self:
+            if x.head is not self and x.through is not self:
                 raise RuntimeError("a fused hidden layer's partial logits reached a layer that is not its head")
             return x
         if x.dim() == 1:
@@ -214,7 +242,9 @@
         x2 = x.reshape(-1, K) if shared else x.reshape(S, -1, K)
         if keys is not None:
             odt = torch.bfloat16 if (self.out_dtype == torch.bfloat16 and mode == "bf16") else torch.float32
-            hp = self._try_fused_head(x2, shared, per, S, mode, predrawn, sample_head=True)
+            hp = self._try_chain(x2, shared, per, S, mode, predrawn)
+            if hp is None:
+                hp = self._try_fused_head(x2, shared, per, S, mode, predrawn, sample_head=True)
             if hp is not None:
                 return hp
             y = ops.linear_sampled(x2, self.weight.mean, self.weight.scale,
diff --git a/bayesianneuralnetworks_amd/ops.py b/bayesianneuralnetworks_amd/ops.py
--- a/bayesianneuralnetworks_amd/ops.py
+++ b/bayesianneuralnetworks_amd/ops.py
@@ -252,10 +252,14 @@
 
 
 class HeadPartials:
-    __slots__ = ("p", "head")
-
-    def __init__(self, p, head=None):
-        self.p, self.head = p, head
+    __slots__ = ("p", "head", "through")
+
+    def __init__(self, p, head=None, through=None):
+        self.p, self.head, self.through = p, head, through
+
+    def _via(self, through, head):
+        self.through, self.head = through, head
+        return self
 
     @property
     def shape(self):
@@ -295,6 +299,63 @@
     check(lib.bnn_dense_forward_head(ptr(x2), x_sample_stride, ldx, ptr(pre.w), N * kp, kp, ptr(pre.b), N if pre.b is not None else 0,
                                      ptr(pre_head.w), Nh * kph, kph, ptr(pre_head.b), Nh if pre_head.b is not None else 0, Nh,
                                      ptr(P), M, N, K, S, _lib.FLAG_RELU if relu else 0, stream_ptr(x2.device)), "bnn_dense_forward_head")
+    return HeadPartials(P)
+
+
+def dense_chain_eligible(M, K1, pre1, pre2, pre_head):
+    if pre1 is None or pre2 is None or pre1.w.dim() != 3 or pre2.w.dim() != 3 or \
+            not dense_head_eligible(M, pre2.w.shape[1], pre2, pre_head):
+        return False
+    S, N1, _ = pre1.w.shape
+    if pre2.w.shape[0] != S or pre2.w.shape[2] < N1 or N1 % 8 != 0:
+        return False
+    return bool(_lib.load().bnn_dense_chain_eligible(M, N1, K1, pre2.w.shape[1], S))
+
+
+_chain_ws = {}
+_chain_pool = {}
+_CHAIN_POOL_WORDS = 1 << 16
+
+
+def _chain_workspace(device, nbytes):
+    words = nbytes // 4
+    if torch.cuda.is_current_stream_capturing():
+        pool = _chain_pool.get(device.index)
+        if pool is not None and pool[1] + words <= pool[0].numel():
+            ws = pool[0][pool[1]:pool[1] + words]
+            pool[1] += (words + 15) // 16 * 16
+            return ws
+        return torch.zeros(words, dtype=torch.int32, device=device)
+    if device.index not in _chain_pool:
+        _chain_pool[device.index] = [torch.zeros(_CHAIN_POOL_WORDS, dtype=torch.int32, device=device), 0]
+    key = (device.index, torch.cuda.current_stream(device).cuda_stream, nbytes)
+    ws = _chain_ws.get(key)
+    if ws is None:
+        ws = _chain_ws[key] = torch.zeros(words, dtype=torch.int32, device=device)
+    return ws
+
+
+def _dense_chain_raw(x2, x_sample_stride, M, pre1, K1, pre2, relu2, pre_head, ldx=None):
+    S, N1, kp1 = pre1.w.shape
+    _, N2, kp2 = pre2.w.shape
+    _, Nh, kph = pre_head.w.shape
+    lib = _lib.load()
+    dev = x2.device
+    ldh = _pad64(N1)
+    h1 = torch.empty((S, M, ldh), dtype=torch.bfloat16, device=dev)
+    parts = lib.bnn_dense_head_parts(M, N2, S)
+    P = torch.empty((parts, S, M, Nh), dtype=torch.float32, device=dev)
+    nb = lib.bnn_dense_chain_workspace_bytes(M, S)
+    ws = _chain_workspace(dev, nb)
+    _lib.ensure_workspace(dev)
+    ldx = K1 if ldx is None else ldx
+    check(lib.bnn_dense_forward_chain(ptr(x2), x_sample_stride, ldx,
+                                      ptr(pre1.w), N1 * kp1, kp1, ptr(pre1.b), N1 if pre1.b is not None else 0,
+                                      ptr(h1), M * ldh, ldh,
+                                      ptr(pre2.w), N2 * kp2, kp2, ptr(pre2.b), N2 if pre2.b is not None else 0,
+                                      ptr(pre_head.w), Nh * kph, kph, ptr(pre_head.b), Nh if pre_head.b is not None else 0, Nh,
+                                      ptr(P), M, N1, K1, N2, S, _lib.FLAG_RELU if relu2 else 0, ptr(ws), nb,
+                                      stream_ptr(dev)), "bnn_dense_forward_chain")
     return HeadPartials(P)
 
 
diff --git a/include/bnn_hip.h b/include/bnn_hip.h
--- a/include/bnn_hip.h
+++ b/include/bnn_hip.h
@@ -131,6 +131,15 @@
                            const void *w_head, int64_t wh_sample_stride, int64_t ldwh,
                            const float *b_head, int64_t bh_sample_stride, int64_t n_head,
                            float *partials, int64_t M, int64_t N, int64_t K, int nsamples, int flags, void *stream);
+int bnn_dense_chain_eligible(int64_t M, int64_t N1, int64_t K1, int64_t N2, int nsamples);
+int64_t bnn_dense_chain_workspace_bytes(int64_t M, int nsamples);
+int bnn_dense_forward_chain(const void *x, int64_t x_sample_stride, int64_t ldx,
+                            const void *w1, int64_t w1_sample_stride, int64_t ldw1, const float *b1, int64_t b1_sample_stride,
+                            void *h1, int64_t h1_sample_stride, int64_t ldh,
+                            const void *w2, int64_t w2_sample_stride, int64_t ldw2, const float *b2, int64_t b2_sample_stride,
+                            const void *w_head, int64_t wh_sample_stride, int64_t ldwh, const float *b_head, int64_t bh_sample_stride,
+                            int64_t n_head, float *partials, int64_t M, int64_t N1, int64_t K1, int64_t N2, int nsamples, int flags,
+                            void *workspace, int64_t workspace_bytes, void *stream);
 int bnn_dense_forward_x3_head(const void *x, int64_t x_plane_stride, int64_t x_sample_stride, int64_t ldx,
                               const void *w, int64_t w_plane_stride, int64_t w_sample_stride, int64_t ldw,
                               const float *b, int64_t b_sample_stride,
```

Result: no change. 202,300, median of 6 (+1.6%).
